# h3poteto/aws-global-accelerator-controller

Hardware: NVIDIA H100
Metric: objects reconciled/sec at 10^6 Service+Ingress; change-set bit-exact vs Go ref (higher is better)
Workload: dtype u8/u32 (bytes and indices)

## Files before the change

### aws-global-accelerator-controller_b200/csrc/gar_pipeline.h

```cpp
#pragma once

#include <stdio.h>
#include <stdlib.h>

#include <initializer_list>

#include "gar_rows.h"

#if defined(__CUDA_ARCH__)
#define GAR_ATOMIC_ADD(p, v) atomicAdd((p), (v))
#else
#define GAR_ATOMIC_ADD(p, v) (*(p) += (v))
#endif


enum Slot {
  S_DERIVED, S_OFLAGS, S_OKEY_HASH, S_STAGE_GA, S_STAGE_R53, S_ANN_R53, S_ANN_NAME, S_ANN_TAGS, S_ANN_LISTEN, S_DPORT_BEGIN, S_DPORTS,
  S_TOK_CODE, S_TOK_NAME, S_TOK_REGION,
  S_ACC_FLAGS, S_ACC_OWNER_KEY, S_ACC_OWNER, S_ACC_THOST, S_ACC_MANAGED, S_ACC_OWNER_HASH, S_ACC_THOST_HASH, S_REC_NAME_HASH, S_VAL_KEY_HASH,
  S_REC_ZONE, S_VAL_REC, S_VAL_CLS, S_VAL_KEY, S_VAL_ORPHAN, S_VAL_LINK, S_ACC_DIGEST,
  S_R53_MODE, S_R53_ACC, S_R53_ACC_DNS, S_PAIR_BEGIN, S_PAIR_OBJ, S_PAIR_HN, S_PAIR_CODE, S_PAIR_ZONE, S_PAIR_REC,
  S_IX_LB, S_IX_OWNER = S_IX_LB + 3, S_IX_THOST = S_IX_OWNER + 3, S_IX_ZONE = S_IX_THOST + 3, S_IX_VAL = S_IX_ZONE + 3,
  S_IX_ALIAS = S_IX_VAL + 3, S_IX_OBJ = S_IX_ALIAS + 3, S_IX_OVN = S_IX_OBJ + 3,
  S_SORT_KEYS = S_IX_OVN + 3, S_SORT_VALS, S_SORT_KEYS_ALT, S_SORT_VALS_ALT, S_SORT_TAGS,
  S_COUNTS, S_STATUS_GA, S_STATUS_R53, S_OPS, S_ERRFLAG, S_IX_EG, S_IX_EG_ENT, S_IX_EG_PAD, S_ACC_CLAIMED,
  S_IXA_BEGIN, S_IXA_FILL, S_IXA_ENT, S_IXA_MULTI, S_OVN_FILL, S_OVN_MULTI, S_LB_HASH, S_REC_FLAGS,
  S_NSLOTS
};


struct FClassify {
  DevTables T;
  Work W;
  u32 *derived_public;
  u8 *oflags;
  u32 *errflag;
  GAR_HD void operator()(u32 i) const {
    classify_object(T, W, i);
    u32 dv = W.derived[i];
    if (dv & OBJ_KEY_BAD) GAR_ATOMIC_ADD(errflag, 1u);
    derived_public[i] = dv & 0xFFu;
  }
};
struct FTokenise {
  DevTables T;
  Work W;
  static constexpr int kStageCols = 1;
  static constexpr u32 kStageBytes = 24 * 1024;
  static constexpr bool kStageByDefault = true;
  GAR_HD void operator()(u32 i) const { tokenise_hostname(T, W, i); }
  GAR_HD const u8 *stage_slab(int) const { return T.o.slab; }
  GAR_HD bool stage_window(int, u32 r0, u32 r1, u64 *lo, u64 *hi) const {
    gar_str a = T.o.lbi_hostname[r0], b = T.o.lbi_hostname[r1 - 1];
    *lo = GAR_STR_OFF(a);
    *hi = GAR_STR_OFF(b) + GAR_STR_LEN(b);
    return true;
  }
  template <class View>
  GAR_HD void run(u32 i, const View &view) const { tokenise_hostname_at(T, W, i, view(0, T.o.lbi_hostname[i])); }
};
struct FDigestAccel {
  DevTables T;
  Work W;
  GAR_HD void operator()(u32 i) const { digest_accelerator(T, W, i); }
};
struct FExpand {
  const u32 *begin;
  u32 nparents;
  u32 *parent_of;
  GAR_HD void operator()(u32 c) const {
    u32 lo = 0, hi = nparents;
    while (hi - lo > 1) {
      u32 mid = (lo + hi) >> 1;
      if (begin[mid] <= c) lo = mid;
      else hi = mid;
    }
    parent_of[c] = lo;
  }
};
constexpr u32 REC_INLINE_VALUES = 32;
constexpr u32 REC_HUGE_VALUES = 4096;
struct DirectView {
  const u8 *slab;
  GAR_HD Str operator()(int, gar_str r) const { return mkstr(slab, r); }
};
struct FPrepareRecord {
  DevTables T;
  Work W;
  u32 *big, *huge;
  static constexpr int kStageCols = 2;
  static constexpr u32 kStageBytes = 16 * 1024;
  static constexpr bool kStageByDefault = true;
  GAR_HD const u8 *stage_slab(int) const { return T.a.slab; }
  GAR_HD bool stage_window(int c, u32 r0, u32 r1, u64 *lo, u64 *hi) const {
    if (c == 0) {
      gar_str a = T.a.rec_name[r0], b = T.a.rec_name[r1 - 1];
      *lo = GAR_STR_OFF(a);
      *hi = GAR_STR_OFF(b) + GAR_STR_LEN(b);
      return true;
    }
    u32 v0 = T.a.rec_val_begin[r0], v1 = T.a.rec_val_begin[r1];
    if (v1 == v0) return false;
    gar_str a = T.a.val_value[v0], b = T.a.val_value[v1 - 1];
    *lo = GAR_STR_OFF(a);
    *hi = GAR_STR_OFF(b) + GAR_STR_LEN(b);
    return true;
  }
  GAR_HD void operator()(u32 r) const { run(r, DirectView{T.a.slab}); }
  template <class View>
  GAR_HD void run(u32 r, const View &view) const {
    u32 lo = 0, hi = T.a.n_zones;
    while (hi - lo > 1) {
      u32 mid = (lo + hi) >> 1;
      if (T.a.zone_rec_begin[mid] <= r) lo = mid;
      else hi = mid;
    }
    W.rec_zone[r] = lo;
    const Str nm = view(0, T.a.rec_name[r]);
    const u64 nh = gar_hash(nm);
    W.rec_name_hash[r] = nh;
    W.rec_flags[r] = find_byte(nm, 0, '\\') < nm.n ? 1 : 0;
    if (T.a.rec_has_alias[r]) ix_count(W.hist[IX_ALIAS], key_hash_zoned_h(lo, nh));
    u32 v0 = T.a.rec_val_begin[r], v1 = T.a.rec_val_begin[r + 1];
    if (v1 - v0 > REC_INLINE_VALUES) {
      u32 *list = v1 - v0 > REC_HUGE_VALUES ? huge : big;
#if defined(__CUDA_ARCH__)
      list[1 + atomicAdd(list, 1u)] = r;
#else
      list[1 + list[0]++] = r;
#endif
      return;
    }
    for (u32 v = v0; v < v1; v++) {
      W.val_rec[v] = r;
      classify_value_at(T, W, v, view(1, T.a.val_value[v]));
    }
  }
};
constexpr u32 BIG_BLOCKS = 528;
struct FClassifyBigRecords {
  DevTables T;
  Work W;
  const u32 *big, *huge;
  GAR_HD void operator()(u32 i) const {
    const u32 blk = i >> 8, tid = i & 255u, nbig = big[0], nhuge = huge[0];
    for (u32 k = blk; k < nbig; k += BIG_BLOCKS) {
      u32 r = big[1 + k];
      for (u32 v = T.a.rec_val_begin[r] + tid; v < T.a.rec_val_begin[r + 1]; v += 256) {
        W.val_rec[v] = r;
        classify_value(T, W, v);
      }
    }
    for (u32 k = 0; k < nhuge; k++) {
      u32 r = huge[1 + k];
      for (u32 v = T.a.rec_val_begin[r] + i; v < T.a.rec_val_begin[r + 1]; v += BIG_BLOCKS * 256) {
        W.val_rec[v] = r;
        classify_value(T, W, v);
      }
    }
  }
};
struct FJsonCount {
  DevTables T;
  Work W;
  GAR_HD void operator()(u32 i) const {
    u32 n = 0;
    if (W.derived[i] & GAR_DV_PORTS_FROM_ANN) {
      u32 stk[GAR_JSON_STACK_WORDS];
      int c = json_listen_ports(mkstr(T.o.slab, W.ann_listen[i]), nullptr, stk);
      n = c < 0 ? 0u : (u32)c;
    }
    W.dport_begin[i] = n;
  }
};
struct FJsonWrite {
  DevTables T;
  Work W;
  GAR_HD void operator()(u32 i) const {
    if (!(W.derived[i] & GAR_DV_PORTS_FROM_ANN)) return;
    if (W.dport_begin[i + 1] == W.dport_begin[i] || W.dport_begin[i + 1] > W.dport_cap) return;
    u32 stk[GAR_JSON_STACK_WORDS];
    json_listen_ports(mkstr(T.o.slab, W.ann_listen[i]), W.dports + W.dport_begin[i], stk);
  }
};

struct FLbHash {
  DevTables T;
  Work W;
  GAR_HD void operator()(u32 i) const {
    u64 h = key_hash_lb(mkstr(T.a.slab, T.a.lb_region[i]), mkstr(T.a.slab, T.a.lb_name[i]));
    W.lb_hash[i] = h;
    ix_count(W.hist[IX_LB], h);
  }
};
struct FRowLb {
  DevTables T;
  Work W;
  GAR_HD bool make(u32 i, u64 *h, IdxEntry *e) const {
    *h = W.lb_hash[i];
    e->a0 = T.a.lb_state[i];
    e->a1 = 0;
    e->s0 = T.a.lb_name[i];
    e->s1 = T.a.lb_region[i];
    return true;
  }
};
struct FRowOwner {
  DevTables T;
  Work W;
  GAR_HD bool make(u32 i, u64 *h, IdxEntry *e) const {
    u32 fl = W.acc_flags[i];
    *h = W.acc_owner_hash[i];
    e->a0 = fl;
    e->a1 = 0;
    e->s0 = W.acc_owner_key[i];
    e->s1 = 0;
    return (fl & ACC_MINE) && (fl & ACC_OWNER_KEYED) && i < W.acc_guest_from;
  }
};
struct FRowThost {
  DevTables T;
  Work W;
  GAR_HD bool make(u32 i, u64 *h, IdxEntry *e) const {
    *h = W.acc_thost_hash[i];
    e->a0 = e->a1 = 0;
    e->s0 = W.acc_thost[i];
    e->s1 = T.a.acc_dns[i];
    return (W.acc_flags[i] & ACC_MINE) != 0 && (!W.sharded || i >= W.acc_guest_from);
  }
};
struct FRowZone {
  DevTables T;
  GAR_HD bool make(u32 i, u64 *h, IdxEntry *e) const {
    Str zn = mkstr(T.a.slab, T.a.zone_name[i]);
    bool valid = zn.n >= 1 && zn.p[zn.n - 1] == '.';
    *h = valid ? key_hash_str(substr(zn, 0, zn.n - 1)) : 0;
    e->a0 = e->a1 = 0;
    e->s0 = T.a.zone_name[i];
    e->s1 = 0;
    return valid;
  }
};
struct FZoneLenMask {
  DevTables T;
  Work W;
  unsigned long long *mask;
  GAR_HD void operator()(u32 z) const {
    Str zn = mkstr(T.a.slab, T.a.zone_name[z]);
    if (zn.n < 1 || zn.p[zn.n - 1] != '.') return;
    ix_count(W.hist[IX_ZONE], key_hash_str(substr(zn, 0, zn.n - 1)));
    u32 b = zn.n - 1 < 255 ? zn.n - 1 : 255;
#if defined(__CUDA_ARCH__)
    atomicOr(&mask[b >> 6], 1ull << (b & 63));
#else
    mask[b >> 6] |= 1ull << (b & 63);
#endif
  }
};
struct FRowVal {
  DevTables T;
  Work W;
  GAR_HD bool make(u32 v, u64 *h, IdxEntry *e) const {
    u32 cls = W.val_cls[v];
    *h = W.val_key_hash[v];
    if (cls == VAL_NOT_OWNER) return false;
    u32 rec = W.val_rec[v];
    u32 kind = (cls & VAL_OWNER_INGRESS) ? 1u : 0u;
    u32 bs = (W.rec_flags[rec] & 1) ? VALNAME_HAS_BACKSLASH : 0u;
    e->a0 = rec;
    e->a1 = W.rec_zone[rec] | bs | (kind << 31);
    e->s0 = W.val_key[v];
    e->s1 = T.a.rec_name[rec];
    return true;
  }
};
struct FRowAlias {
  DevTables T;
  Work W;
  GAR_HD bool make(u32 r, u64 *h, IdxEntry *e) const {
    *h = key_hash_zoned_h(W.rec_zone[r], W.rec_name_hash[r]);
    e->a0 = W.rec_zone[r];
    e->a1 = T.a.rec_type[r];
    e->s0 = T.a.rec_name[r];
    e->s1 = T.a.rec_alias_dns[r];
    return T.a.rec_has_alias[r] != 0;
  }
};
struct FRowObj {
  DevTables T;
  Work W;
  GAR_HD bool make(u32 i, u64 *h, IdxEntry *e) const {
    gar_str ns = T.o.obj_ns[i];
    *h = W.okey_hash[i];
    e->a0 = T.o.obj_kind[i];
    e->a1 = 0;
    e->s0 = GAR_STR(GAR_STR_OFF(ns), GAR_STR_LEN(ns) + 1 + GAR_STR_LEN(T.o.obj_name[i]));
    e->s1 = 0;
    return !(W.derived[i] & OBJ_KEY_BAD);
  }
};
struct FRowOvn {
  DevTables T;
  Work W;
  GAR_HD bool make(u32 v, u64 *h, IdxEntry *e) const {
    u32 rec = W.val_rec[v];
    *h = key_hash_zoned_h(W.rec_zone[rec], W.rec_name_hash[rec]);
    e->a0 = rec;
    e->a1 = W.rec_zone[rec];
    e->s0 = T.a.rec_name[rec];
    e->s1 = T.a.val_value[v];
    return W.val_orphan[v] != 0;
  }
};

constexpr u32 IDX_SMALL_BUCKET = 48;
template <class RowF>
struct FIdxRows {
  RowF rowf;
  u32 *keys, *vals;
  IdxEntry *tmp;
  u32 *counts;
  u32 mask, nb;
  GAR_HD void operator()(u32 i) const {
    u64 h = 0;
    IdxEntry e;
    bool valid = rowf.make(i, &h, &e);
    u32 k = valid ? hash_bucket(h, mask) : nb;
    keys[i] = k;
    if (vals) vals[i] = i;
    if (valid) {
      e.tag = hash_tag(h);
      e.row = i;
      tmp[i] = e;
      GAR_ATOMIC_ADD(&counts[k], 1u);
    }
  }
};
struct FIdxPlace {
  const u32 *keys;
  u32 *cursor;
  const IdxEntry *tmp;
  IdxEntry *ent;
  u32 nb;
  GAR_HD void operator()(u32 i) const {
    u32 k = keys[i];
    if (k == nb) return;
#if defined(__CUDA_ARCH__)
    u32 pos = atomicAdd(&cursor[k], 1u);
#else
    u32 pos = cursor[k]++;
#endif
    ent[pos] = tmp[i];
  }
};
struct FIdxOrder {
  const u32 *begin;
  IdxEntry *ent;
  u32 *overflow;
  GAR_HD void operator()(u32 b) const {
    u32 lo = begin[b], m = begin[b + 1] - lo;
    if (m < 2) return;
    if (m > IDX_SMALL_BUCKET) {
      GAR_ATOMIC_ADD(overflow, 1u);
      return;
    }
    for (u32 k = 1; k < m; k++) {
      IdxEntry x = ent[lo + k];
      u32 j = k;
      while (j > 0 && ent[lo + j - 1].row > x.row) {
        ent[lo + j] = ent[lo + j - 1];
        j--;
      }
      if (j != k) ent[lo + j] = x;
    }
  }
};
struct FIdxGather {
  const u32 *vals;
  const u32 *nvalid;
  const IdxEntry *tmp;
  IdxEntry *ent;
  GAR_HD void operator()(u32 p) const {
    if (p < *nvalid) ent[p] = tmp[vals[p]];
  }
};
template <class RowF>
struct FIdxPlaceDirect {
  RowF rowf;
  u32 *cursor;
  IdxEntry *ent;
  u32 mask;
  GAR_HD void operator()(u32 i) const {
    u64 h = 0;
    IdxEntry e;
    if (!rowf.make(i, &h, &e)) return;
    const u32 k = hash_bucket(h, mask);
#if defined(__CUDA_ARCH__)
    const u32 pos = atomicAdd(&cursor[k], 1u);
#else
    const u32 pos = cursor[k]++;
#endif
    e.tag = hash_tag(h);
    e.row = i;
    ent[pos] = e;
  }
};
struct FIdxMultiList {
  const u32 *begin;
  u32 *multi;
  GAR_HD void operator()(u32 b) const {
    const bool m = begin[b + 1] - begin[b] >= 2;
#if defined(__CUDA_ARCH__)
    const unsigned active = __activemask();
    const unsigned votes = __ballot_sync(active, m);
    if (!m) return;
    const unsigned lane = threadIdx.x & 31u;
    const int leader = __ffs(votes) - 1;
    u32 base = 0;
    if ((int)lane == leader) base = atomicAdd(multi, (u32)__popc(votes));
    base = __shfl_sync(votes, base, leader);
    multi[1 + base + __popc(votes & ((1u << lane) - 1u))] = b;
#else
    if (m) multi[1 + multi[0]++] = b;
#endif
  }
};
struct FIdxOrderMulti {
  const u32 *begin;
  IdxEntry *ent;
  const u32 *multi;
  u32 *overflow;
  GAR_HD void operator()(u32 t) const {
    const u32 b = multi[1 + t];
    const u32 lo = begin[b], m = begin[b + 1] - lo;
    if (m > IDX_SMALL_BUCKET) {
      GAR_ATOMIC_ADD(overflow, 1u);
      return;
    }
    for (u32 k = 1; k < m; k++) {
      IdxEntry x = ent[lo + k];
      u32 j = k;
      while (j > 0 && ent[lo + j - 1].row > x.row) {
        ent[lo + j] = ent[lo + j - 1];
        j--;
      }
      if (j != k) ent[lo + j] = x;
    }
  }
};
enum FlagWord { FW_BAD_KEYS = 0, FW_IDX_OVERFLOW = 1, FW_NDPORTS = 2, FW_NPAIRS = 3, FW_SEC0 = 4 , FW_WORDS = 16 };
struct FGatherFinal {
  const u32 *src;
  u32 idx[5];
  const u32 *npairs;
  u32 *flags;
  GAR_HD void operator()(u32 k) const {
    if (k < 5) flags[FW_SEC0 + k] = src[idx[k]];
    else if (npairs) flags[FW_NPAIRS] = *npairs;
  }
};
struct FGather5 {
  const u32 *src;
  u32 idx[5];
  const u32 *extra;
  u32 *dst;
  GAR_HD void operator()(u32 k) const { dst[k] = k < 5 ? src[idx[k]] : *extra; }
};
#define GAR_RETRY_WITH_RADIX 1000
#define GAR_REFUSE_EMPTY_CACHE 1001
struct FGatherHeader {
  const u32 *ndports;
  u32 *flags;
  GAR_HD void operator()(u32) const { flags[FW_NDPORTS] = *ndports; }
};
struct FValueJoins {
  DevTables T;
  Work W;
  GAR_HD void operator()(u32 v) const {
    link_value_alias(T, W, v);
    mark_orphan_value(T, W, v);
  }
};
struct FMarkOrphanValue {
  DevTables T;
  Work W;
  GAR_HD void operator()(u32 v) const { mark_orphan_value(T, W, v); }
};

struct CountLayout {
  u32 n, nacc, nrec, nval;
  GAR_HD u32 ga_obj(u32 i) const { return i; }
  GAR_HD u32 ga_orph(u32 a) const { return n + a; }
  GAR_HD u32 r53_obj(u32 i) const { return n + nacc + i; }
  GAR_HD u32 base0() const { return 2 * n + nacc; }
  GAR_HD u32 base1() const { return 2 * n + nacc + nrec; }
  GAR_HD u32 total() const { return 2 * n + nacc + nrec + nval; }
};
constexpr u32 OPS_STAGE_CAP = 4;
struct FGaObj {
  DevTables T;
  Work W;
  u32 *counts;
  gar_op *stage;
  u32 *status;
  const u32 *rows;
  GAR_HD void operator()(u32 t, bool valid) const {
    u32 i = (rows && valid) ? rows[t] : t;
    OpSink s{stage + (size_t)t * OPS_STAGE_CAP, 0, OPS_STAGE_CAP};
    u32 st = ga_reconcile(T, W, i, valid, s);
    if (valid) {
      status[t] = st;
      counts[t] = s.n;
    }
  }
};
struct FR53Obj {
  DevTables T;
  Work W;
  u32 *counts;
  gar_op *stage;
  u32 *status;
  const u32 *rows;
  GAR_HD void operator()(u32 t, bool valid) const {
    u32 i = (rows && valid) ? rows[t] : t;
    OpSink s{stage + (size_t)t * OPS_STAGE_CAP, 0, OPS_STAGE_CAP};
    u32 prev = (valid && W.r53_mode[i] == R53_MODE_DONE) ? status[t] : 0;
    u32 st = r53_combine(T, W, i, t, valid, prev, s);
    if (valid) {
      status[t] = st;
      counts[t] = s.n;
    }
  }
};
struct FR53Prepare {
  DevTables T;
  Work W;
  u32 *status;
  const u32 *rows;
  GAR_HD void operator()(u32 t, bool valid) const { r53_prepare(T, W, (rows && valid) ? rows[t] : t, t, valid, status); }
};
struct FR53FillPairs {
  DevTables T;
  Work W;
  const u32 *rows;
  GAR_HD void operator()(u32 t) const { r53_fill_pairs(T, W, rows ? rows[t] : t, t); }
};
struct FR53Pair {
  DevTables T;
  Work W;
  GAR_HD void operator()(u32 p, bool valid) const { r53_pair(T, W, p, valid); }
};
struct DelKeys {
  const u8 *kind;
  const gar_str *key;
  const u8 *slab;
};
struct FDelKeyGa {
  DevTables T;
  Work W;
  DelKeys D;
  u32 *counts;
  gar_op *ops;
  u32 cap;
  GAR_HD void operator()(u32 k) const {
    u32 kind = D.kind[k];
    Str key = mkstr(D.slab, D.key[k]);
    if (ops && counts[k + 1] > cap) return;
    OpSink s{ops ? ops + counts[k] : nullptr, 0, 0xFFFFFFFFu};
    OwnerIter it = owner_open(W, key_hash_kinded(kind, key), key);
    for (u32 acc; (acc = owner_next(T, W, kind, it)) != GAR_NONE;) put_delete_chain(T, s, GAR_NONE, 0, acc);
    if (!ops) counts[k] = s.n;
  }
};
struct FDelKeyR53 {
  DevTables T;
  Work W;
  DelKeys D;
  u32 *counts;
  gar_op *ops;
  u32 cap;
  GAR_HD void operator()(u32 k) const {
    u32 kind = D.kind[k];
    Str key = mkstr(D.slab, D.key[k]);
    if (ops && counts[k + 1] > cap) return;
    OpSink s{ops ? ops + counts[k] : nullptr, 0, 0xFFFFFFFFu};
    Owned ow;
    owned_collect(T, W, key_hash_kinded(kind, key), kind, key, ow);
    r53_cleanup(T, W, GAR_NONE, 0, ow, s);
    if (!ops) counts[k] = s.n;
  }
};
struct FRowKnownEg {
  gar_bindings b;
  GAR_HD bool make(u32 i, u64 *h, IdxEntry *e) const {
    *h = gar_hash(mkstr(b.slab, b.known_eg_arn[i]));
    e->a0 = e->a1 = 0;
    e->s0 = b.known_eg_arn[i];
    e->s1 = 0;
    return true;
  }
};
struct FEgb {
  DevTables T;
  Work W;
  DevBindings B;
  u32 *counts;
  gar_op *ops;
  u32 *status;
  u32 cap;
  GAR_HD void operator()(u32 k) const {
    if (ops && counts[k + 1] > cap) return;
    OpSink s{ops ? ops + counts[k] : nullptr, 0, 0xFFFFFFFFu};
    u32 st = egb_reconcile(T, W, B, k, s);
    if (ops) status[k] = st;
    else counts[k] = s.n;
  }
};
struct FGatherDerived {
  const u32 *derived, *rows;
  u32 *out;
  GAR_HD void operator()(u32 t) const { out[t] = derived[rows[t]] & 0xFFu; }
};
struct FCompactOps {
  DevTables T;
  Work W;
  const u32 *scanned;
  const gar_op *stage;
  gar_op *ops;
  u32 ctrl;
  const u32 *rows;
  u32 cap;
  GAR_HD void operator()(u32 t, bool valid) const {
    u32 i = (rows && valid) ? rows[t] : t;
    u32 off = 0, c = 0;
    if (valid) {
      off = scanned[t];
      c = scanned[t + 1] - off;
      if (off > cap || c > cap - off) c = 0;
      if (c <= OPS_STAGE_CAP)
        for (u32 k = 0; k < c; k++) ops[off + k] = stage[(size_t)t * OPS_STAGE_CAP + k];
    }
    bool redo = valid && c > OPS_STAGE_CAP;
    if (GAR_ANY(redo)) {
      OpSink s{ops + off, 0, redo ? c : 0u};
      if (ctrl == GAR_CTRL_GA) ga_reconcile(T, W, i, redo, s);
      else r53_reconcile(T, W, i, redo, s);
    }
  }
};
struct FGaOrphan {
  DevTables T;
  Work W;
  CountLayout L;
  u32 *counts;
  gar_op *ops;
  u32 cap;
  GAR_HD void operator()(u32 a) const {
    if (ops && counts[L.ga_orph(a) + 1] == counts[L.ga_orph(a)]) return;
    if (ops && counts[L.ga_orph(a) + 1] > cap) return;
    OpSink s{ops ? ops + counts[L.ga_orph(a)] : nullptr, 0, 0xFFFFFFFFu};
    ga_orphan(T, W, a, s);
    if (!ops) counts[L.ga_orph(a)] = s.n;
  }
};
struct FR53OrphanAlias {
  DevTables T;
  Work W;
  CountLayout L;
  u32 *counts;
  gar_op *ops;
  u32 cap;
  GAR_HD void operator()(u32 r) const {
    if (!ops) {
      OpSink s{nullptr, 0, 0};
      r53_orphan_alias(T, W, r, s);
      counts[L.base0() + r] = s.n;
      return;
    }
    if (counts[L.base0() + r + 1] == counts[L.base0() + r]) return;
    if (counts[L.total()] > cap) return;
    u32 z = W.rec_zone[r];
    u32 zv = T.a.rec_val_begin[T.a.zone_rec_begin[z]];
    u32 off = counts[L.base0()] + (counts[L.base1() + zv] - counts[L.base1()]) + (counts[L.base0() + r] - counts[L.base0()]);
    OpSink s{ops + off, 0, 0xFFFFFFFFu};
    r53_orphan_alias(T, W, r, s);
  }
};
struct FR53OrphanValue {
  DevTables T;
  Work W;
  CountLayout L;
  u32 *counts;
  gar_op *ops;
  u32 cap;
  GAR_HD void operator()(u32 v) const {
    if (!ops) {
      counts[L.base1() + v] = W.val_orphan[v];
      return;
    }
    if (!W.val_orphan[v] || counts[L.total()] > cap) return;
    u32 r = W.val_rec[v];
    u32 z = W.rec_zone[r];
    u32 rend = T.a.zone_rec_begin[z + 1];
    u32 off = counts[L.base0()] + (counts[L.base0() + rend] - counts[L.base0()]) + (counts[L.base1() + v] - counts[L.base1()]);
    gar_op o;
    o.head = GAR_OP_HEAD(GAR_OP_R53_DELETE_RECORD, GAR_CTRL_R53, 0);
    o.obj = GAR_NONE;
    o.sub = 1;
    o.a0 = z;
    o.a1 = r;
    o.a2 = v;
    ops[off] = o;
  }
};


struct DiffCounts {
  u64 n_ops;
  u64 section_begin[GAR_N_SECTIONS + 1];
  u64 n_dports;
  u32 bad_keys;
};

GAR_HD u32 next_pow2(u32 x) {
  u32 p = 1;
  while (p < x) p <<= 1;
  return p;
}
inline int ilog2(u32 p) {
  int b = 0;
  while ((1u << b) < p) b++;
  return b;
}

template <class B>
struct Pipeline {
  B &be;
  DevTables T;
  Work W{};
  bool force_radix = false;
  explicit Pipeline(B &b, const DevTables &t) : be(b), T(t) {}

  template <class RowF>
  HashIdx build_index(int slot, u32 nrows, u32 load, RowF rowf, u32 *overflow, bool force_radix) {
    u32 nb = next_pow2(nrows / load < 16 ? 16 : nrows / load);
    u32 *keys = (u32 *)be.ensure(S_SORT_KEYS, sizeof(u32) * (size_t)(nrows + 1));
    u32 *vals = (u32 *)be.ensure(S_SORT_VALS, sizeof(u32) * (size_t)(nrows + 1));
    IdxEntry *tmp = (IdxEntry *)be.ensure(S_SORT_TAGS, sizeof(IdxEntry) * (size_t)(nrows + 1));
    u32 *begin = (u32 *)be.ensure(slot + 0, sizeof(u32) * (size_t)(nb + 2));
    IdxEntry *ent = (IdxEntry *)be.ensure(slot + 1, sizeof(IdxEntry) * (size_t)(nrows + 1));
    be.fill32(begin, 0, nb + 2);
    if (nrows) be.for_each("idx_rows", nrows, FIdxRows<RowF>{rowf, keys, force_radix ? vals : nullptr, tmp, begin, nb - 1, nb});
    be.exclusive_scan(begin, nb + 2);
    if (nrows && !force_radix) {
      u32 *cursor = (u32 *)be.ensure(S_SORT_KEYS_ALT, sizeof(u32) * (size_t)(nb + 1));
      be.copy32(cursor, begin, nb);
      be.for_each("idx_place", nrows, FIdxPlace{keys, cursor, tmp, ent, nb});
      be.for_each("idx_order", nb, FIdxOrder{begin, ent, overflow});
    } else if (nrows) {
      u32 *keys2 = (u32 *)be.ensure(S_SORT_KEYS_ALT, sizeof(u32) * (size_t)(nrows + 1));
      u32 *vals2 = (u32 *)be.ensure(S_SORT_VALS_ALT, sizeof(u32) * (size_t)(nrows + 1));
      be.sort_pairs(keys, vals, keys2, vals2, nrows, ilog2(nb) + 1);
      be.for_each("idx_gather", nrows, FIdxGather{vals, begin + nb, tmp, ent});
    }
    return HashIdx{begin, ent, nb - 1};
  }

  bool prepared = false;
  u64 n_dports = 0;
  u32 *errflag = nullptr;

  u32 acc_guest_from = 0xFFFFFFFFu;
  u32 sharded = 0;
  bool orphan_sweep = true;
  bool allow_empty_cache = false;

  void alloc_obj_work() {
    const u32 n = T.o.n_objects, nlbi = T.o.n_lbi;
    W.derived = (u32 *)be.ensure(S_DERIVED, 4 * (size_t)(n + 1));
    W.okey_hash = (u64 *)be.ensure(S_OKEY_HASH, 8 * (size_t)(n + 1));
    W.ann_r53 = (gar_str *)be.ensure(S_ANN_R53, 8 * (size_t)(n + 1));
    W.ann_name = (gar_str *)be.ensure(S_ANN_NAME, 8 * (size_t)(n + 1));
    W.ann_tags = (gar_str *)be.ensure(S_ANN_TAGS, 8 * (size_t)(n + 1));
    W.ann_listen = (gar_str *)be.ensure(S_ANN_LISTEN, 8 * (size_t)(n + 1));
    W.dport_begin = (u32 *)be.out_dport_begin(n);
    W.tok_code = (u8 *)be.out_tok_code(nlbi);
    W.tok_name = (gar_str *)be.out_tok_name(nlbi);
    W.tok_region = (gar_str *)be.out_tok_region(nlbi);
    W.r53_mode = (u8 *)be.ensure(S_R53_MODE, (size_t)n + 1);
    W.r53_acc = (u32 *)be.ensure(S_R53_ACC, 4 * (size_t)(n + 1));
    W.r53_acc_dns = (gar_str *)be.ensure(S_R53_ACC_DNS, 8 * (size_t)(n + 1));
  }
  void alloc_work() {
    const u32 nacc = T.a.n_accels, nrec = T.a.n_records, nval = T.a.n_values;
    alloc_obj_work();
    W.acc_flags = (u32 *)be.ensure(S_ACC_FLAGS, 4 * (size_t)(nacc + 1));
    W.acc_owner_key = (gar_str *)be.ensure(S_ACC_OWNER_KEY, 8 * (size_t)(nacc + 1));
    W.acc_owner = (gar_str *)be.ensure(S_ACC_OWNER, 8 * (size_t)(nacc + 1));
    W.acc_thost = (gar_str *)be.ensure(S_ACC_THOST, 8 * (size_t)(nacc + 1));
    W.acc_managed = (gar_str *)be.ensure(S_ACC_MANAGED, 8 * (size_t)(nacc + 1));
    W.acc_owner_hash = (u64 *)be.ensure(S_ACC_OWNER_HASH, 8 * (size_t)(nacc + 1));
    W.acc_thost_hash = (u64 *)be.ensure(S_ACC_THOST_HASH, 8 * (size_t)(nacc + 1));
    W.rec_name_hash = (u64 *)be.ensure(S_REC_NAME_HASH, 8 * (size_t)(nrec + 1));
    W.val_key_hash = (u64 *)be.ensure(S_VAL_KEY_HASH, 8 * (size_t)(nval + 1));
    W.rec_zone = (u32 *)be.ensure(S_REC_ZONE, 4 * (size_t)(nrec + 1));
    W.val_rec = (u32 *)be.ensure(S_VAL_REC, 4 * (size_t)(nval + 1));
    W.val_cls = (u8 *)be.ensure(S_VAL_CLS, nval + 1);
    W.val_key = (gar_str *)be.ensure(S_VAL_KEY, 8 * (size_t)(nval + 1));
    W.val_orphan = (u8 *)be.ensure(S_VAL_ORPHAN, nval + 1);
    W.val_link = (ValLink *)be.ensure(S_VAL_LINK, sizeof(ValLink) * (size_t)(nval + 1));
    W.acc_digest = (AccDigest *)be.ensure(S_ACC_DIGEST, sizeof(AccDigest) * (size_t)(nacc + 1));
    W.lb_hash = (u64 *)be.ensure(S_LB_HASH, 8 * (size_t)(T.a.n_lbs + 1));
    W.rec_flags = (u8 *)be.ensure(S_REC_FLAGS, (size_t)nrec + 1);
    for (int k = 0; k < IX_N; k++) W.hist[k] = IxHist{nullptr, 0};
    W.pair_cap = 0;
    W.dport_cap = 0;
    errflag = (u32 *)be.ensure(S_ERRFLAG, 256);
    be.fill32(errflag, 0, FW_WORDS);
    W.acc_guest_from = acc_guest_from;
    W.sharded = sharded;
    W.acc_claimed = nullptr;
  }
  void stage1() {
    const u32 n = T.o.n_objects, nlbi = T.o.n_lbi, nacc = T.a.n_accels, nrec = T.a.n_records, nval = T.a.n_values;
    u32 *derived_public = (u32 *)be.out_derived(n);
    if (n) be.for_each("classify_objects", n, FClassify{T, W, derived_public, nullptr, errflag});
    if (nlbi) be.for_each_staged("tokenise_hostnames", nlbi, FTokenise{T, W});
    if (nacc) be.for_each("digest_accelerators", nacc, FDigestAccel{T, W});
    if (T.a.n_lbs) be.for_each("hash_load_balancers", T.a.n_lbs, FLbHash{T, W});
    {
      unsigned long long *zm = (unsigned long long *)(errflag + 16 + 8);
      be.fill32((u32 *)zm, 0, 8);
      if (T.a.n_zones) be.for_each("zone_len_mask", T.a.n_zones, FZoneLenMask{T, W, zm});
      W.zone_len_mask = (const u64 *)zm;
    }
    if (nrec) {
      u32 *big = (u32 *)be.ensure(S_SORT_KEYS, 4 * (size_t)(nval / REC_INLINE_VALUES + 2));
      u32 *huge = (u32 *)be.ensure(S_SORT_VALS, 4 * (size_t)(nval / REC_HUGE_VALUES + 2));
      be.fill32(big, 0, 1);
      be.fill32(huge, 0, 1);
      be.for_each_staged("prepare_records", nrec, FPrepareRecord{T, W, big, huge});
      if (nval > REC_INLINE_VALUES) be.for_each("prepare_records", BIG_BLOCKS * 256, FClassifyBigRecords{T, W, big, huge});
    }
  }
  struct IxPlan {
    u32 off[IX_N] = {}, nb[IX_N] = {}, rows[IX_N] = {};
    bool want[IX_N] = {};
    u32 total_nb = 0;
    u64 total_rows = 0;
  };
  IxPlan planA;
  u32 *ixa_begin = nullptr, *ixa_fill = nullptr, *ixa_multi = nullptr;
  IdxEntry *ixa_ent = nullptr;
  u32 ovn_nb = 0;
  void arm_group_a(u32 want_mask) {
    const u32 rows[IX_N] = {T.a.n_lbs, T.a.n_accels, T.a.n_accels, T.a.n_zones, T.a.n_values, T.a.n_records, T.o.n_objects, 0};
    const u32 load[IX_N] = {1, 1, 1, 1, 1, 2, 1, 8};
    planA = IxPlan{};
    for (int k = 0; k < IX_OVN; k++) {
      planA.want[k] = (want_mask >> k) & 1u;
      if (!planA.want[k]) continue;
      planA.rows[k] = rows[k];
      planA.nb[k] = next_pow2(rows[k] / load[k] < 16 ? 16 : rows[k] / load[k]);
      planA.off[k] = planA.total_nb;
      planA.total_nb += planA.nb[k];
      planA.total_rows += rows[k];
    }
    ixa_begin = (u32 *)be.ensure(S_IXA_BEGIN, 4 * (size_t)(planA.total_nb + 2));
    be.fill32(ixa_begin, 0, (size_t)planA.total_nb + 2);
    for (int k = 0; k < IX_OVN; k++)
      if (planA.want[k]) W.hist[k] = IxHist{ixa_begin + planA.off[k], planA.nb[k] - 1};
  }
  HashIdx group_a_index(int k) const { return HashIdx{ixa_begin + planA.off[k], ixa_ent, planA.nb[k] - 1}; }
  template <class RowF>
  FIdxPlaceDirect<RowF> placer(int k, RowF rowf) const {
    return FIdxPlaceDirect<RowF>{rowf, ixa_fill + planA.off[k], ixa_ent, planA.nb[k] - 1};
  }
  void finish_group_a() {
    u32 *overflow = errflag + FW_IDX_OVERFLOW;
    be.exclusive_scan(ixa_begin, planA.total_nb + 1);
    ixa_fill = (u32 *)be.ensure(S_IXA_FILL, 4 * (size_t)(planA.total_nb + 1));
    ixa_ent = (IdxEntry *)be.ensure(S_IXA_ENT, sizeof(IdxEntry) * (size_t)(planA.total_rows + 1));
    const u32 multi_cap = (u32)(planA.total_rows / 2 + 1);
    ixa_multi = (u32 *)be.ensure(S_IXA_MULTI, 4 * (size_t)(multi_cap + 2));
    be.copy32(ixa_fill, ixa_begin, (size_t)planA.total_nb + 1);
    be.fill32(ixa_multi, 0, 1);
    const IxPlan &P = planA;
    auto n = [&](int k) { return P.want[k] ? P.rows[k] : 0u; };
    be.for_each_multi("idx_place", {n(IX_LB), n(IX_OWNER), n(IX_THOST), n(IX_ZONE), n(IX_VAL), n(IX_ALIAS), n(IX_OBJ), P.total_nb},
                      placer(IX_LB, FRowLb{T, W}), placer(IX_OWNER, FRowOwner{T, W}), placer(IX_THOST, FRowThost{T, W}), placer(IX_ZONE, FRowZone{T}),
                      placer(IX_VAL, FRowVal{T, W}), placer(IX_ALIAS, FRowAlias{T, W}), placer(IX_OBJ, FRowObj{T, W}), FIdxMultiList{ixa_begin, ixa_multi});
    be.for_each_dyn("idx_order", ixa_multi, multi_cap, FIdxOrderMulti{ixa_begin, ixa_ent, ixa_multi, overflow});
    if (P.want[IX_LB]) W.ix_lb = group_a_index(IX_LB);
    if (P.want[IX_OWNER]) W.ix_owner = group_a_index(IX_OWNER);
    if (P.want[IX_THOST]) W.ix_thost = group_a_index(IX_THOST);
    if (P.want[IX_ZONE]) W.ix_zone = group_a_index(IX_ZONE);
    if (P.want[IX_VAL]) W.ix_val = group_a_index(IX_VAL);
    if (P.want[IX_ALIAS]) W.ix_alias = group_a_index(IX_ALIAS);
    if (P.want[IX_OBJ]) W.ix_obj = group_a_index(IX_OBJ);
  }
  void arm_ovn() {
    ovn_nb = next_pow2(T.a.n_values / 8 < 16 ? 16 : T.a.n_values / 8);
    u32 *cnt = (u32 *)be.ensure(S_IX_OVN + 0, 4 * (size_t)(ovn_nb + 2));
    be.fill32(cnt, 0, (size_t)ovn_nb + 2);
    W.hist[IX_OVN] = IxHist{cnt, ovn_nb - 1};
  }
  void finish_ovn() {
    const u32 nval = T.a.n_values;
    u32 *begin = W.hist[IX_OVN].cnt;
    be.exclusive_scan(begin, ovn_nb + 1);
    u32 *cursor = (u32 *)be.ensure(S_OVN_FILL, 4 * (size_t)(ovn_nb + 1));
    IdxEntry *ent = (IdxEntry *)be.ensure(S_IX_OVN + 1, sizeof(IdxEntry) * (size_t)(nval + 1));
    u32 *multi = (u32 *)be.ensure(S_OVN_MULTI, 4 * (size_t)(nval / 2 + 3));
    be.copy32(cursor, begin, (size_t)ovn_nb + 1);
    be.fill32(multi, 0, 1);
    be.for_each_multi("idx_place", {nval, ovn_nb}, FIdxPlaceDirect<FRowOvn>{FRowOvn{T, W}, cursor, ent, ovn_nb - 1}, FIdxMultiList{begin, multi});
    be.for_each_dyn("idx_order", multi, nval / 2 + 1, FIdxOrderMulti{begin, ent, multi, errflag + FW_IDX_OVERFLOW});
    W.ix_ovn = HashIdx{begin, ent, ovn_nb - 1};
  }

  void prepare_route() {
    alloc_work();
    arm_group_a(1u << IX_ALIAS);
    stage1();
    finish_group_a();
  }
  void prepare_directory() {
    alloc_work();
    arm_group_a((1u << IX_LB) | (1u << IX_THOST));
    if (T.o.n_lbi) be.for_each("tokenise_hostnames", T.o.n_lbi, FTokenise{T, W});
    if (T.a.n_accels) be.for_each("digest_accelerators", T.a.n_accels, FDigestAccel{T, W});
    if (T.a.n_lbs) be.for_each("hash_load_balancers", T.a.n_lbs, FLbHash{T, W});
    finish_group_a();
  }

  u32 dport_cap = 0, pair_cap = 0;
  u64 ops_cap = 0;
  bool tiny_caps = false;
  int prepare() {
    const u32 n = T.o.n_objects, nacc = T.a.n_accels, nzone = T.a.n_zones, nrec = T.a.n_records, nval = T.a.n_values;
    alloc_work();
    if (!force_radix) {
      arm_group_a((1u << IX_OVN) - 1);
      arm_ovn();
    }
    stage1();
    listen_ports();

    u32 *overflow = errflag + FW_IDX_OVERFLOW;
    if (!force_radix) {
      finish_group_a();
      if (nval) be.for_each("value_joins", nval, FValueJoins{T, W});
      finish_ovn();
    } else {
      W.ix_lb = build_index(S_IX_LB, T.a.n_lbs, 1, FRowLb{T, W}, overflow, true);
      W.ix_owner = build_index(S_IX_OWNER, nacc, 1, FRowOwner{T, W}, overflow, true);
      W.ix_thost = build_index(S_IX_THOST, nacc, 1, FRowThost{T, W}, overflow, true);
      W.ix_zone = build_index(S_IX_ZONE, nzone, 1, FRowZone{T}, overflow, true);
      W.ix_val = build_index(S_IX_VAL, nval, 1, FRowVal{T, W}, overflow, true);
      W.ix_alias = build_index(S_IX_ALIAS, nrec, 2, FRowAlias{T, W}, overflow, true);
      W.ix_obj = build_index(S_IX_OBJ, n, 1, FRowObj{T, W}, overflow, true);
      if (nval) be.for_each("value_joins", nval, FValueJoins{T, W});
      W.ix_ovn = build_index(S_IX_OVN, nval, 8, FRowOvn{T, W}, overflow, true);
    }
    obj_stale = ovn_stale = false;
    return GAR_OK;
  }
  void listen_ports() {
    const u32 n = T.o.n_objects;
    be.fill32(W.dport_begin, 0, (size_t)n + 1);
    if (n) be.for_each("listen_ports_count", n, FJsonCount{T, W});
    be.exclusive_scan(W.dport_begin, n + 1);
    be.for_each("gather_header", 1, FGatherHeader{W.dport_begin + n, errflag});
    if (dport_cap < n / 2 + 1024 && !(tiny_caps && dport_cap)) dport_cap = tiny_caps ? 1 : n / 2 + 1024;
    W.dport_cap = dport_cap;
    W.dports = (i32 *)be.out_dports(dport_cap);
    if (n) be.for_each("listen_ports_write", n, FJsonWrite{T, W});
  }

  bool obj_stale = false, ovn_stale = false;
  void prepare_objects() {
    const u32 n = T.o.n_objects, nlbi = T.o.n_lbi;
    alloc_obj_work();
    be.fill32(errflag, 0, FW_WORDS);
    W.hist[IX_OBJ] = IxHist{nullptr, 0};
    u32 *derived_public = (u32 *)be.out_derived(n);
    if (n) be.for_each("classify_objects", n, FClassify{T, W, derived_public, nullptr, errflag});
    if (nlbi) be.for_each_staged("tokenise_hostnames", nlbi, FTokenise{T, W});
    listen_ports();
    W.ix_obj = build_index(S_IX_OBJ, n, 1, FRowObj{T, W}, errflag + FW_IDX_OVERFLOW, force_radix);
    obj_stale = false;
    ovn_stale = true;
  }
  void prepare_orphan_values() {
    const u32 nval = T.a.n_values;
    if (!force_radix) {
      arm_ovn();
      if (nval) be.for_each("orphan_values", nval, FMarkOrphanValue{T, W});
      finish_ovn();
    } else {
      W.hist[IX_OVN] = IxHist{nullptr, 0};
      if (nval) be.for_each("orphan_values", nval, FMarkOrphanValue{T, W});
      W.ix_ovn = build_index(S_IX_OVN, nval, 8, FRowOvn{T, W}, errflag + FW_IDX_OVERFLOW, true);
    }
    ovn_stale = false;
  }
  int index_objects() {
    for (int attempt = 0; attempt < 2; attempt++) {
      if (!prepared) prepare();
      else if (obj_stale) prepare_objects();
      prepared = true;
      u32 fl[FW_WORDS];
      be.download(fl, errflag, sizeof(fl));
      if (fl[FW_BAD_KEYS]) return GAR_E_INVALID;
      if (fl[FW_IDX_OVERFLOW] && !force_radix) {
        force_radix = true;
        prepared = false;
        continue;
      }
      return GAR_OK;
    }
    return GAR_E_STATE;
  }

  u64 n_pairs = 0;
  void r53_relational(u32 slots, const u32 *rows, u32 *st_r53) {
    W.pair_begin = (u32 *)be.ensure(S_PAIR_BEGIN, 4 * (size_t)(slots + 2));
    be.fill32(W.pair_begin, 0, (size_t)slots + 1);
    if (slots) be.for_each_warp("r53_prepare", slots, FR53Prepare{T, W, st_r53, rows});
    be.exclusive_scan(W.pair_begin, slots + 1);
    if (pair_cap < slots + slots / 2 + 1024 && !(tiny_caps && pair_cap)) pair_cap = tiny_caps ? 1 : slots + slots / 2 + 1024;
    W.pair_cap = pair_cap;
    W.pair_obj = (u32 *)be.ensure(S_PAIR_OBJ, 4 * (size_t)(pair_cap + 1));
    W.pair_hn = (gar_str *)be.ensure(S_PAIR_HN, 8 * (size_t)(pair_cap + 1));
    W.pair_code = (u8 *)be.ensure(S_PAIR_CODE, (size_t)pair_cap + 1);
    W.pair_zone = (u32 *)be.ensure(S_PAIR_ZONE, 4 * (size_t)(pair_cap + 1));
    W.pair_rec = (u32 *)be.ensure(S_PAIR_REC, 4 * (size_t)(pair_cap + 1));
    if (slots) {
      be.for_each("r53_fill_pairs", slots, FR53FillPairs{T, W, rows});
      be.for_each_warp_dyn("r53_pairs", W.pair_begin + slots, pair_cap, FR53Pair{T, W});
    }
  }

  template <class OpsAlloc>
  int decide_all(OpsAlloc ops_alloc) {
    const u32 n = T.o.n_objects, nacc = T.a.n_accels, nrec = T.a.n_records, nval = T.a.n_values;
    CountLayout L{n, nacc, nrec, nval};
    u32 *counts = (u32 *)be.ensure(S_COUNTS, 4 * (size_t)(L.total() + 2));
    be.fill32(counts, 0, (size_t)L.total() + 1);
    gar_op *stage_ga = (gar_op *)be.ensure(S_STAGE_GA, sizeof(gar_op) * ((size_t)n * OPS_STAGE_CAP + 1));
    gar_op *stage_r53 = (gar_op *)be.ensure(S_STAGE_R53, sizeof(gar_op) * ((size_t)n * OPS_STAGE_CAP + 1));
    u32 *st_ga = (u32 *)be.out_status_ga(n);
    u32 *st_r53 = (u32 *)be.out_status_r53(n);
    W.acc_claimed = (u8 *)be.ensure(S_ACC_CLAIMED, (size_t)nacc + 4);
    be.fill32((u32 *)W.acc_claimed, 0, ((size_t)nacc + 3) / 4);
    if (n) be.for_each_warp("ga_objects", n, FGaObj{T, W, counts + L.ga_obj(0), stage_ga, st_ga, nullptr});
    r53_relational(n, nullptr, st_r53);
    if (n) be.for_each_warp("r53_objects", n, FR53Obj{T, W, counts + L.r53_obj(0), stage_r53, st_r53, nullptr});
    if (orphan_sweep)
      be.for_each_multi("orphans_count", {nacc, nrec, nval}, FGaOrphan{T, W, L, counts, nullptr, 0}, FR53OrphanAlias{T, W, L, counts, nullptr, 0},
                        FR53OrphanValue{T, W, L, counts, nullptr, 0});
    be.exclusive_scan(counts, L.total() + 1);
    be.for_each("gather_section_begins", 6, FGatherFinal{counts, {0, L.ga_orph(0), L.r53_obj(0), L.base0(), L.total()}, W.pair_begin + n, errflag});

    const u64 est = tiny_caps ? 1 : (u64)n + nacc / 8 + 1024;
    if (ops_cap < est) ops_cap = est;
    gar_op *ops = (gar_op *)ops_alloc(ops_cap);
    const u32 cap = ops_cap > 0xFFFFFFF0ull ? 0xFFFFFFF0u : (u32)ops_cap;
    if (n) be.for_each_warp("ga_objects_compact", n, FCompactOps{T, W, counts + L.ga_obj(0), stage_ga, ops, GAR_CTRL_GA, nullptr, cap});
    if (n) be.for_each_warp("r53_objects_compact", n, FCompactOps{T, W, counts + L.r53_obj(0), stage_r53, ops, GAR_CTRL_R53, nullptr, cap});
    if (orphan_sweep)
      be.for_each_multi("orphans_emit", {nacc, nrec, nval}, FGaOrphan{T, W, L, counts, ops, cap}, FR53OrphanAlias{T, W, L, counts, ops, cap},
                        FR53OrphanValue{T, W, L, counts, ops, cap});
    W.acc_claimed = nullptr;
    return GAR_OK;
  }

  template <class OpsAlloc>
  int decide_keys(const u32 *rows, u32 m, DelKeys D, u32 nd, OpsAlloc ops_alloc) {
    const u32 total = 2 * m + 2 * nd;
    u32 *counts = (u32 *)be.ensure(S_COUNTS, 4 * (size_t)(total + 2));
    be.fill32(counts, 0, (size_t)total + 1);
    u32 *c_ga = counts, *c_gad = counts + m, *c_r53 = counts + m + nd, *c_r53d = counts + 2 * m + nd;
    gar_op *stage_ga = (gar_op *)be.ensure(S_STAGE_GA, sizeof(gar_op) * ((size_t)m * OPS_STAGE_CAP + 1));
    gar_op *stage_r53 = (gar_op *)be.ensure(S_STAGE_R53, sizeof(gar_op) * ((size_t)m * OPS_STAGE_CAP + 1));
    u32 *st_ga = (u32 *)be.out_status_ga(m);
    u32 *st_r53 = (u32 *)be.out_status_r53(m);
    u32 *derived_out = (u32 *)be.out_derived_keys(m);
    if (m) {
      be.for_each("gather_derived", m, FGatherDerived{W.derived, rows, derived_out});
      be.for_each_warp("ga_objects", m, FGaObj{T, W, c_ga, stage_ga, st_ga, rows});
    }
    if (nd) be.for_each("ga_deleted_keys_count", nd, FDelKeyGa{T, W, D, c_gad, nullptr, 0});
    r53_relational(m, rows, st_r53);
    if (m) be.for_each_warp("r53_objects", m, FR53Obj{T, W, c_r53, stage_r53, st_r53, rows});
    if (nd) be.for_each("r53_deleted_keys_count", nd, FDelKeyR53{T, W, D, c_r53d, nullptr, 0});
    be.exclusive_scan(counts, total + 1);
    be.for_each("gather_section_begins", 6, FGatherFinal{counts, {0, m, m + nd, 2 * m + nd, total}, W.pair_begin + m, errflag});
    const u64 est = tiny_caps ? 1 : 2 * (u64)m + 4 * (u64)nd + 256;
    if (ops_cap < est) ops_cap = est;
    gar_op *ops = (gar_op *)ops_alloc(ops_cap);
    const u32 cap = ops_cap > 0xFFFFFFF0ull ? 0xFFFFFFF0u : (u32)ops_cap;
    if (m) be.for_each_warp("ga_objects_compact", m, FCompactOps{T, W, c_ga, stage_ga, ops, GAR_CTRL_GA, rows, cap});
    if (nd) be.for_each("ga_deleted_keys_emit", nd, FDelKeyGa{T, W, D, c_gad, ops, cap});
    if (m) be.for_each_warp("r53_objects_compact", m, FCompactOps{T, W, c_r53, stage_r53, ops, GAR_CTRL_R53, rows, cap});
    if (nd) be.for_each("r53_deleted_keys_emit", nd, FDelKeyR53{T, W, D, c_r53d, ops, cap});
    return GAR_OK;
  }

  template <class OpsAlloc>
  int decide_bindings(const gar_bindings &b, OpsAlloc ops_alloc) {
    u32 *overflow = errflag + FW_IDX_OVERFLOW;
    const u32 nb = b.n_bindings;
    DevBindings DB{b, build_index(S_IX_EG, b.n_known_egs, 1, FRowKnownEg{b}, overflow, force_radix)};
    u32 *counts = (u32 *)be.ensure(S_COUNTS, 4 * (size_t)(nb + 2));
    be.fill32(counts, 0, (size_t)nb + 1);
    u32 *st = (u32 *)be.out_status_ga(nb);
    if (nb) be.for_each("egb_count", nb, FEgb{T, W, DB, counts, nullptr, nullptr, 0});
    be.exclusive_scan(counts, nb + 1);
    be.for_each("gather_section_begins", 6, FGatherFinal{counts, {0, nb, nb, nb, nb}, nullptr, errflag});
    const u64 est = tiny_caps ? 1 : 4 * (u64)nb + 256;
    if (ops_cap < est) ops_cap = est;
    gar_op *ops = (gar_op *)ops_alloc(ops_cap);
    const u32 cap = ops_cap > 0xFFFFFFF0ull ? 0xFFFFFFF0u : (u32)ops_cap;
    if (nb) be.for_each("egb_emit", nb, FEgb{T, W, DB, counts, ops, st, cap});
    return GAR_OK;
  }

  template <class DecideF>
  int run_with(DiffCounts *dc, bool full, DecideF decide) {
    for (int attempt = 0; attempt < 8; attempt++) {
      u64 sig = 0;
      if (full) {
        sig = hmix(hmix(prepared ? (obj_stale || ovn_stale ? 9 : 1) : 2, force_radix ? 3 : 4), hmix(hmix(dport_cap, pair_cap), ops_cap));
        sig = hmix(sig, hmix(orphan_sweep ? 5 : 6, tiny_caps ? 7 : 8)) | 1;
      }
      const int g = full ? be.graph_begin(sig) : 0;
      int rc = GAR_OK;
      if (g != 2) {
        if (!prepared) rc = prepare();
        else if (obj_stale) prepare_objects();
        if (rc == GAR_OK && full && ovn_stale) prepare_orphan_values();
        if (rc == GAR_OK) rc = decide();
      }
      prepared = true;
      if (full) be.graph_end();
      if (rc != GAR_OK) return rc;
      u32 fl[FW_WORDS];
      be.download(fl, errflag, sizeof(fl));
      if (fl[FW_BAD_KEYS]) return GAR_E_INVALID;
      if (fl[FW_IDX_OVERFLOW] && !force_radix) {
        force_radix = true;
        prepared = false;
        continue;
      }
      if (fl[FW_NDPORTS] > dport_cap) {
        dport_cap = fl[FW_NDPORTS] + fl[FW_NDPORTS] / 8 + 16;
        prepared = false;
        continue;
      }
      if (fl[FW_NPAIRS] > pair_cap) {
        pair_cap = fl[FW_NPAIRS] + fl[FW_NPAIRS] / 8 + 16;
        continue;
      }
      const u64 nops = fl[FW_SEC0 + 4];
      if (nops > ops_cap) {
        ops_cap = nops + nops / 8 + 16;
        continue;
      }
      n_dports = fl[FW_NDPORTS];
      n_pairs = fl[FW_NPAIRS];
      for (int k = 0; k < 5; k++) dc->section_begin[k] = fl[FW_SEC0 + k];
      dc->n_ops = nops;
      dc->n_dports = full ? n_dports : 0;
      if (full && T.o.n_objects == 0 && !sharded && !allow_empty_cache && nops != 0) return GAR_REFUSE_EMPTY_CACHE;
      return GAR_OK;
    }
    return GAR_E_STATE;
  }
  template <class OpsAlloc>
  int run(DiffCounts *dc, OpsAlloc ops_alloc) {
    return run_with(dc, true, [&] { return decide_all(ops_alloc); });
  }
  template <class OpsAlloc>
  int run_keys(const u32 *rows, u32 m, DelKeys D, u32 nd, DiffCounts *dc, OpsAlloc ops_alloc) {
    return run_with(dc, false, [&] { return decide_keys(rows, m, D, nd, ops_alloc); });
  }
  template <class OpsAlloc>
  int run_bindings(const gar_bindings &b, DiffCounts *dc, OpsAlloc ops_alloc) {
    return run_with(dc, false, [&] { return decide_bindings(b, ops_alloc); });
  }
};
```

### aws-global-accelerator-controller_b200/csrc/gar_rows.h

```cpp
#pragma once

#include "gar_common.h"
#include "gar_json.h"


struct DevTables {
  gar_objects o;
  gar_actual a;
  const u8 *cluster;
  u32 cluster_len;
};

enum {
  OBJ_HAS_NAME_ANN = 1u << 8,
  OBJ_HAS_TAGS_ANN = 1u << 9,
  OBJ_KEY_BAD = 1u << 10,
};

enum {
  ACC_MINE = 1u << 0,
  ACC_OWNER_KEYED = 1u << 1,
  ACC_OWNER_INGRESS = 1u << 2,
  ACC_OWNER_3PART = 1u << 3,
  ACC_HAS_MANAGED = 1u << 4, ACC_HAS_OWNER = 1u << 5, ACC_HAS_THOST = 1u << 6,
};

enum {
  R53_MODE_DONE = 0,
  R53_MODE_PAIRS = 1,
  R53_MODE_OBJECT = 2,
};
enum { PAIR_IN_SYNC = 0, PAIR_CREATE = 1, PAIR_UPSERT = 2, PAIR_NO_ZONE = 3,
       PAIR_REPEAT = 4 };
#define VALNAME_HAS_BACKSLASH (1u << 30)

enum { VAL_NOT_OWNER = 0, VAL_OWNER_SERVICE = 1, VAL_OWNER_INGRESS = 2, VAL_OWNER_3PART = 4 };

struct alignas(64) AccDigest {
  u32 flags;
  u32 lis;
  u32 eg;
  u32 pr_begin;
  u32 ep_begin;
  u16 n_ports, n_eps;
  i32 port0, port1;
  gar_str name;
  gar_str thost;
  gar_str owner_key;
  gar_str ep0;
};
enum {
  ACCD_ENABLED = 1u << 8,
  ACCD_MANAGED_TRUE = 1u << 9,
  ACCD_LIS_NONE = 1u << 10, ACCD_LIS_MANY = 1u << 11,
  ACCD_LIS_UDP = 1u << 12,
  ACCD_EG_NONE = 1u << 13, ACCD_EG_MANY = 1u << 14,
};
struct alignas(16) ValLink {
  u32 alias_row, pad;
  gar_str alias_dns;
};

enum IxId { IX_LB, IX_OWNER, IX_THOST, IX_ZONE, IX_VAL, IX_ALIAS, IX_OBJ, IX_OVN, IX_N };
struct IxHist {
  u32 *cnt;
  u32 mask;
};
#if defined(__CUDA_ARCH__)
#define GAR_HIST_ADD(p) atomicAdd((p), 1u)
#else
#define GAR_HIST_ADD(p) (++*(p))
#endif
GAR_HD void ix_count(const IxHist &h, u64 key_hash) {
  if (h.cnt) GAR_HIST_ADD(&h.cnt[(u32)key_hash & h.mask]);
}

struct Work {
  IxHist hist[IX_N];
  u64 *lb_hash;
  u8 *rec_flags;
  u32 pair_cap;
  u32 dport_cap;
  u32 *derived;
  u64 *okey_hash;
  gar_str *ann_r53;
  gar_str *ann_name;
  gar_str *ann_tags;
  gar_str *ann_listen;
  u32 *dport_begin;
  i32 *dports;
  u8 *tok_code;
  gar_str *tok_name, *tok_region;
  u32 *acc_flags;
  gar_str *acc_owner_key;
  gar_str *acc_owner;
  gar_str *acc_thost;
  gar_str *acc_managed;
  AccDigest *acc_digest;
  u64 *acc_owner_hash;
  u64 *acc_thost_hash;
  u32 *rec_zone;
  u64 *rec_name_hash;
  u32 *val_rec;
  u8 *val_cls;
  gar_str *val_key;
  u64 *val_key_hash;
  u8 *val_orphan;
  ValLink *val_link;
  u32 acc_guest_from;
  u32 sharded;
  u8 *acc_claimed;
  u8 *r53_mode;
  u32 *r53_acc;
  gar_str *r53_acc_dns;
  u32 *pair_begin;
  u32 *pair_obj;
  gar_str *pair_hn;
  u8 *pair_code;
  u32 *pair_zone;
  u32 *pair_rec;
  HashIdx ix_lb;
  HashIdx ix_owner;
  HashIdx ix_thost;
  HashIdx ix_zone;
  const u64 *zone_len_mask;
  HashIdx ix_val;
  HashIdx ix_alias;
  HashIdx ix_obj;
  HashIdx ix_ovn;
};

GAR_HD bool acc_in_owner_index(const Work &W, u32 a, u32 fl) { return (fl & ACC_MINE) && (fl & ACC_OWNER_KEYED) && a < W.acc_guest_from; }
GAR_HD bool acc_in_thost_index(const Work &W, u32 a, u32 fl) { return (fl & ACC_MINE) != 0 && (!W.sharded || a >= W.acc_guest_from); }


GAR_HD u64 key_hash_kinded(u32 kind, Str nsname) { return hmix(kind + 1, gar_hash(nsname)); }
GAR_HD u64 key_hash_lb(Str region, Str name) { return hmix(gar_hash(region), gar_hash(name)); }
GAR_HD u64 key_hash_zoned_h(u32 zone, u64 name_hash) { return hmix((u64)zone + 0x100, name_hash); }
GAR_HD u64 key_hash_zoned(u32 zone, Str name) { return key_hash_zoned_h(zone, gar_hash(name)); }
GAR_HD u64 key_hash_str(Str s) { return gar_hash(s); }

GAR_HD Str object_key(const DevTables &T, u32 i) {
  gar_str ns = T.o.obj_ns[i], nm = T.o.obj_name[i];
  return Str{T.o.slab + GAR_STR_OFF(ns), GAR_STR_LEN(ns) + 1 + GAR_STR_LEN(nm)};
}
GAR_HD bool object_key_ok(const DevTables &T, u32 i) {
  gar_str ns = T.o.obj_ns[i], nm = T.o.obj_name[i];
  u64 sep = GAR_STR_OFF(ns) + GAR_STR_LEN(ns);
  return GAR_STR_OFF(nm) == sep + 1 && sep < T.o.slab_len && T.o.slab[sep] == '/';
}


#define ANN_PREFIX "aws-global-accelerator-controller.h3poteto.dev/"

GAR_HD bool proto_is(Str p, char a, char b, char c) {
  return p.n == 3 && (p.p[0] | 0x20) == a && (p.p[1] | 0x20) == b && (p.p[2] | 0x20) == c;
}

GAR_HD void classify_object(const DevTables &T, const Work &W, u32 i) {
  const gar_objects &o = T.o;
  u32 kind = o.obj_kind[i];
  u32 dv = 0;
  bool has_lbtype = false, has_ingclass = false;
  gar_str r53 = 0, name = 0, tags = 0, listen = 0;
  bool has_listen = false;
  for (u32 k = o.obj_ann_begin[i]; k < o.obj_ann_begin[i + 1]; k++) {
    Str key = mkstr(o.slab, o.ann_key[k]);
    gar_str vref = o.ann_val[k];
    if (HAS_PREFIX_LIT(key, ANN_PREFIX)) {
      Str t = substr(key, sizeof(ANN_PREFIX) - 1, key.n - (u32)(sizeof(ANN_PREFIX) - 1));
      if (STREQ_LIT(t, "global-accelerator-managed")) {
        dv |= GAR_DV_GA_MANAGED;
      } else if (STREQ_LIT(t, "route53-hostname")) {
        dv |= GAR_DV_R53_ANNOTATED;
        r53 = vref;
      } else if (STREQ_LIT(t, "client-ip-preservation")) {
        if (STREQ_LIT(mkstr(o.slab, vref), "true")) dv |= GAR_DV_IP_PRESERVE;
        else dv &= ~(u32)GAR_DV_IP_PRESERVE;
      } else if (STREQ_LIT(t, "global-accelerator-name")) {
        dv |= OBJ_HAS_NAME_ANN;
        name = vref;
      } else if (STREQ_LIT(t, "global-accelerator-tags")) {
        dv |= OBJ_HAS_TAGS_ANN;
        tags = vref;
      } else if (STREQ_LIT(t, "ip-address-type")) {
        Str v = mkstr(o.slab, vref);
        if (STREQ_LIT(v, "ipv4") || STREQ_LIT(v, "IPV4")) dv |= GAR_DV_IPV4;
        else dv &= ~(u32)GAR_DV_IPV4;
      }
    } else if (STREQ_LIT(key, "service.beta.kubernetes.io/aws-load-balancer-type")) {
      has_lbtype = true;
    } else if (STREQ_LIT(key, "kubernetes.io/ingress.class")) {
      has_ingclass = true;
    } else if (STREQ_LIT(key, "alb.ingress.kubernetes.io/listen-ports")) {
      has_listen = true;
      listen = vref;
    }
  }
  if (kind == GAR_KIND_SERVICE) {
    bool lbsvc = o.obj_spec_type[i] == GAR_SVC_LOADBALANCER && (has_lbtype || (o.obj_flags[i] & GAR_OBJ_HAS_LB_CLASS));
    if (lbsvc) dv |= GAR_DV_GA_ELIGIBLE | GAR_DV_R53_ELIGIBLE;
    bool udp = false;
    for (u32 p = o.obj_port_begin[i]; p < o.obj_port_begin[i + 1]; p++) {
      Str pr = mkstr(o.slab, o.port_proto[p]);
      if (proto_is(pr, 'u', 'd', 'p')) udp = true;
      else if (proto_is(pr, 't', 'c', 'p')) udp = false;
    }
    if (udp) dv |= GAR_DV_PROTO_UDP;
  } else {
    bool alb = has_ingclass;
    if ((o.obj_flags[i] & GAR_OBJ_HAS_INGRESS_CLASS) && STREQ_LIT(mkstr(o.slab, o.obj_ingress_class[i]), "alb")) alb = true;
    if (alb) dv |= GAR_DV_GA_ELIGIBLE;
    dv |= GAR_DV_R53_ELIGIBLE;
    if (has_listen) dv |= GAR_DV_PORTS_FROM_ANN;
  }
  if (!object_key_ok(T, i)) dv |= OBJ_KEY_BAD;
  const u64 okh = (dv & OBJ_KEY_BAD) ? 0 : key_hash_kinded(kind, object_key(T, i));
  W.okey_hash[i] = okh;
  if (!(dv & OBJ_KEY_BAD)) ix_count(W.hist[IX_OBJ], okh);
  W.derived[i] = dv;
  W.ann_r53[i] = r53;
  W.ann_name[i] = name;
  W.ann_tags[i] = tags;
  W.ann_listen[i] = listen;
}


GAR_HD u32 name_dash_id(Str s) {
  u32 last = GAR_NONE;
  for (u32 i = 0; i < s.n; i += 8) {
    u64 w = load_word(s, i);
    u64 pad = s.n - i < 8 ? ~lowmask(s.n - i) & 0x8080808080808080ull : 0;
    if (w & 0x8080808080808080ull) return 0;
    u64 dash = swar_eq_exact(w, '-') & ~pad;
    u64 ok = swar_in_range(w, '0', '9') | swar_in_range(w, 'A', 'Z') | swar_in_range(w, 'a', 'z') | swar_eq_exact(w, '_') | dash | pad;
    if (ok != 0x8080808080808080ull) return 0;
    if (dash) last = i + ((63 - clz64(dash)) >> 3);
  }
  if (last == GAR_NONE || last < 1 || last + 1 >= s.n) return 0;
  return last;
}

GAR_HD u8 tokenise_str(Str h, u64 base, gar_str *name_out, gar_str *region_out) {
  u8 code;
  gar_str name = 0, region = 0;
  u32 d1 = find_byte(h, 0, '.');
  u32 d2 = d1 < h.n ? find_byte(h, d1 + 1, '.') : h.n;
  u32 d3 = d2 < h.n ? find_byte(h, d2 + 1, '.') : h.n;
  if (d1 >= h.n) {
    code = GAR_TOK_PANIC;
  } else if (!(STREQ_LIT(h, "amazonaws.com") || HAS_SUFFIX_LIT(h, ".amazonaws.com"))) {
    code = GAR_TOK_NOT_AWS;
  } else if (HAS_SUFFIX_LIT(h, ".elb.amazonaws.com")) {
    Str sub = substr(h, 0, d1);
    region = GAR_STR(base + d1 + 1, d2 - d1 - 1);
    if (HAS_PREFIX_LIT(sub, "internal-")) {
      u32 g = name_dash_id(substr(sub, 9, sub.n - 9));
      if (g) {
        code = GAR_TOK_ALB_INTERNAL;
        name = GAR_STR(base + 9, g);
      } else {
        code = GAR_TOK_ERR_INTERNAL_ALB;
      }
    } else {
      u32 g = name_dash_id(sub);
      if (g) {
        code = GAR_TOK_ALB_PUBLIC;
        name = GAR_STR(base, g);
      } else {
        code = GAR_TOK_ERR_PUBLIC_ALB;
      }
    }
  } else {
    bool nlb = false;
    if (h.n >= 20) {
      u32 last = GAR_NONE;
      for (u32 i = d1; i <= h.n - 20; i = find_byte(h, i + 1, '.'))
        if (lit_eq_at(h, i, ".elb.")) last = i;
      if (last != GAR_NONE) nlb = find_byte(substr(h, 0, h.n - 14), last + 5, '\n') >= h.n - 14;
    }
    if (!nlb) {
      code = GAR_TOK_ERR_NOT_ELB;
    } else {
      u32 g = name_dash_id(substr(h, 0, d1));
      if (g) {
        code = GAR_TOK_NLB;
        name = GAR_STR(base, g);
        region = GAR_STR(base + d2 + 1, d3 - d2 - 1);
      } else {
        code = GAR_TOK_ERR_NLB;
      }
    }
  }
  if (code > GAR_TOK_NLB) {
    name = 0;
    region = 0;
  }
  *name_out = name;
  *region_out = region;
  return code;
}
GAR_HD void tokenise_hostname_at(const DevTables &T, const Work &W, u32 row, Str h) {
  gar_str name, region;
  u8 code = tokenise_str(h, GAR_STR_OFF(T.o.lbi_hostname[row]), &name, &region);
  W.tok_code[row] = code;
  W.tok_name[row] = name;
  W.tok_region[row] = region;
}
GAR_HD void tokenise_hostname(const DevTables &T, const Work &W, u32 row) { tokenise_hostname_at(T, W, row, mkstr(T.o.slab, T.o.lbi_hostname[row])); }


#define TAG_MANAGED "aws-global-accelerator-controller-managed"
#define TAG_OWNER "aws-global-accelerator-owner"
#define TAG_THOST "aws-global-accelerator-target-hostname"
#define TAG_CLUSTER "aws-global-accelerator-cluster"

GAR_HD u32 count_slashes(Str s) { return count_byte(s, '/'); }

GAR_HD void digest_accelerator(const DevTables &T, const Work &W, u32 a) {
  const gar_actual &A = T.a;
  gar_str managed = 0, owner = 0, thost = 0, cluster = 0;
  u32 fl = 0;
  for (u32 t = A.acc_tag_begin[a]; t < A.acc_tag_begin[a + 1]; t++) {
    Str k = mkstr(A.slab, A.tag_key[t]);
    if (STREQ_LIT(k, TAG_MANAGED)) {
      managed = A.tag_val[t];
      fl |= ACC_HAS_MANAGED;
    } else if (STREQ_LIT(k, TAG_OWNER)) {
      owner = A.tag_val[t];
      fl |= ACC_HAS_OWNER;
    } else if (STREQ_LIT(k, TAG_THOST)) {
      thost = A.tag_val[t];
      fl |= ACC_HAS_THOST;
    } else if (STREQ_LIT(k, TAG_CLUSTER)) {
      cluster = A.tag_val[t];
    }
  }
  Str cl = mkstr(A.slab, cluster);
  if (STREQ_LIT(mkstr(A.slab, managed), "true") && streq(cl, Str{T.cluster, T.cluster_len})) fl |= ACC_MINE;
  Str ow = mkstr(A.slab, owner);
  gar_str key = 0;
  if (HAS_PREFIX_LIT(ow, "service/")) {
    fl |= ACC_OWNER_KEYED;
    key = GAR_STR(GAR_STR_OFF(owner) + 8, ow.n - 8);
  } else if (HAS_PREFIX_LIT(ow, "ingress/")) {
    fl |= ACC_OWNER_KEYED | ACC_OWNER_INGRESS;
    key = GAR_STR(GAR_STR_OFF(owner) + 8, ow.n - 8);
  }
  if ((fl & ACC_OWNER_KEYED) && count_slashes(mkstr(A.slab, key)) == 1) fl |= ACC_OWNER_3PART;
  AccDigest d;
  d.flags = fl | (A.acc_enabled[a] ? ACCD_ENABLED : 0) | (STREQ_LIT(mkstr(A.slab, managed), "true") ? ACCD_MANAGED_TRUE : 0);
  d.lis = d.eg = d.pr_begin = d.ep_begin = 0;
  d.n_ports = d.n_eps = 0;
  d.port0 = d.port1 = 0;
  d.ep0 = 0;
  u32 lb = A.acc_lis_begin[a], le = A.acc_lis_begin[a + 1];
  if (le == lb) d.flags |= ACCD_LIS_NONE;
  else if (le - lb > 1) d.flags |= ACCD_LIS_MANY;
  else {
    d.lis = lb;
    if (A.lis_proto[lb] == GAR_PROTO_UDP) d.flags |= ACCD_LIS_UDP;
    d.pr_begin = A.lis_pr_begin[lb];
    u32 np = A.lis_pr_begin[lb + 1] - d.pr_begin;
    d.n_ports = (u16)(np > 0xFFFF ? 0xFFFF : np);
    if (np > 0) d.port0 = A.pr_from[d.pr_begin];
    if (np > 1) d.port1 = A.pr_from[d.pr_begin + 1];
    u32 eb = A.lis_eg_begin[lb], ee = A.lis_eg_begin[lb + 1];
    if (ee == eb) d.flags |= ACCD_EG_NONE;
    else if (ee - eb > 1) d.flags |= ACCD_EG_MANY;
    else {
      d.eg = eb;
      d.ep_begin = A.eg_ep_begin[eb];
      u32 ne = A.eg_ep_begin[eb + 1] - d.ep_begin;
      d.n_eps = (u16)(ne > 0xFFFF ? 0xFFFF : ne);
      if (ne > 0) d.ep0 = A.ep_id[d.ep_begin];
    }
  }
  d.name = A.acc_name[a];
  d.thost = thost;
  d.owner_key = key;
  W.acc_digest[a] = d;
  const u64 owner_hash = (fl & ACC_OWNER_KEYED) ? key_hash_kinded((fl & ACC_OWNER_INGRESS) ? 1u : 0u, mkstr(A.slab, key)) : 0;
  const u64 thost_hash = (fl & ACC_MINE) ? gar_hash(mkstr(A.slab, thost)) : 0;
  W.acc_owner_hash[a] = owner_hash;
  W.acc_thost_hash[a] = thost_hash;
  if (acc_in_owner_index(W, a, fl)) ix_count(W.hist[IX_OWNER], owner_hash);
  if (acc_in_thost_index(W, a, fl)) ix_count(W.hist[IX_THOST], thost_hash);
  W.acc_flags[a] = fl;
  W.acc_owner_key[a] = key;
  W.acc_owner[a] = owner;
  W.acc_thost[a] = thost;
  W.acc_managed[a] = managed;
}


#define R53_HERITAGE "\"heritage=aws-global-accelerator-controller,cluster="

GAR_HD void classify_value_at(const DevTables &T, const Work &W, u32 v, Str s) {
  const gar_actual &A = T.a;
  gar_str ref = A.val_value[v];
  u8 cls = VAL_NOT_OWNER;
  gar_str key = 0;
  const u32 hl = (u32)(sizeof(R53_HERITAGE) - 1);
  u32 fixed = hl + T.cluster_len + 1 + 8 + 1;
  if (s.n >= fixed && HAS_PREFIX_LIT(s, R53_HERITAGE) && streq(substr(s, hl, T.cluster_len), Str{T.cluster, T.cluster_len}) &&
      s.p[hl + T.cluster_len] == ',' && s.p[s.n - 1] == '"') {
    u32 ro = hl + T.cluster_len + 1;
    Str rest = substr(s, ro, s.n - 1 - ro);
    if (HAS_PREFIX_LIT(rest, "service/")) cls = VAL_OWNER_SERVICE;
    else if (HAS_PREFIX_LIT(rest, "ingress/")) cls = VAL_OWNER_INGRESS;
    if (cls) {
      key = GAR_STR(GAR_STR_OFF(ref) + ro + 8, rest.n - 8);
      if (count_slashes(substr(rest, 8, rest.n - 8)) == 1) cls |= VAL_OWNER_3PART;
    }
  }
  W.val_cls[v] = cls;
  W.val_key[v] = key;
  const u64 vkh = cls ? key_hash_kinded((cls & VAL_OWNER_INGRESS) ? 1u : 0u, substr(s, (u32)(GAR_STR_OFF(key) - GAR_STR_OFF(ref)), (u32)GAR_STR_LEN(key))) : 0;
  W.val_key_hash[v] = vkh;
  if (cls) ix_count(W.hist[IX_VAL], vkh);
}
GAR_HD void classify_value(const DevTables &T, const Work &W, u32 v) { classify_value_at(T, W, v, mkstr(T.a.slab, T.a.val_value[v])); }


GAR_HD u32 find_lb(const DevTables &T, const Work &W, Str region, Str name, u32 *state) {
  Cursor c = idx_open(W.ix_lb, key_hash_lb(region, name));
  IdxEntry e;
  while (idx_next(W.ix_lb, c, &e))
    if (streq(mkstr(T.a.slab, e.s0), name) && streq(mkstr(T.a.slab, e.s1), region)) {
      *state = e.a0;
      return e.row;
    }
  return GAR_NONE;
}

struct OwnerIter {
  Cursor c;
  Str key;
};
GAR_HD OwnerIter owner_open(const Work &W, u64 key_hash, Str key) { return OwnerIter{idx_open(W.ix_owner, key_hash), key}; }
GAR_HD u32 owner_next(const DevTables &T, const Work &W, u32 kind, OwnerIter &it) {
  IdxEntry e;
  while (idx_next(W.ix_owner, it.c, &e)) {
    if ((((e.a0 & ACC_OWNER_INGRESS) != 0) ? 1u : 0u) != kind) continue;
    if (streq(mkstr(T.a.slab, e.s0), it.key)) return e.row;
  }
  return GAR_NONE;
}

GAR_HD u32 find_by_hostname(const DevTables &T, const Work &W, Str hostname, u32 *first, gar_str *first_dns) {
  Cursor c = idx_open(W.ix_thost, key_hash_str(hostname));
  u32 n = 0;
  *first = GAR_NONE;
  IdxEntry e;
  while (idx_next(W.ix_thost, c, &e)) {
    if (!streq(mkstr(T.a.slab, e.s0), hostname)) continue;
    if (n == 0) {
      *first = e.row;
      *first_dns = e.s1;
    }
    if (++n >= 2) break;
  }
  return n;
}

GAR_HD bool zone_len_possible(const Work &W, u32 n) {
  u32 b = n < 255 ? n : 255;
  return (W.zone_len_mask[b >> 6] >> (b & 63)) & 1ull;
}
GAR_HD u32 find_hosted_zone(const DevTables &T, const Work &W, Str hostname) {
  Str t = hostname;
  for (;;) {
    if (t.n == 0) return GAR_NONE;
    if (zone_len_possible(W, t.n)) {
      Cursor c = idx_open(W.ix_zone, key_hash_str(t));
      IdxEntry e;
      while (idx_next(W.ix_zone, c, &e)) {
        Str zn = mkstr(T.a.slab, e.s0);
        if (zn.n == t.n + 1 && streq(substr(zn, 0, t.n), t)) return e.row;
      }
    }
    u32 k = find_byte(t, 0, '.');
    if (k >= t.n) return GAR_NONE;
    t = substr(t, k + 1, t.n - k - 1);
  }
}

GAR_HD bool record_name_matches(Str name, Str hostname) {
  u32 w = GAR_NONE;
  for (u32 k = find_byte(name, 0, '\\'); k + 4 <= name.n; k = find_byte(name, k + 1, '\\'))
    if (name.p[k + 1] == '0' && name.p[k + 2] == '5' && name.p[k + 3] == '2') {
      w = k;
      break;
    }
  if (w == GAR_NONE) return name.n == hostname.n + 1 && name.p[name.n - 1] == '.' && streq(substr(name, 0, hostname.n), hostname);
  if (name.n - 3 != hostname.n + 1) return false;
  if (name.p[name.n - 1] != '.') return false;
  if (w >= hostname.n || hostname.p[w] != '*') return false;
  if (!streq(substr(name, 0, w), substr(hostname, 0, w))) return false;
  u32 tail = hostname.n - w - 1;
  return streq(substr(name, w + 4, tail), substr(hostname, w + 1, tail));
}


GAR_HD Cursor cursor_none() { return Cursor{0, 0, 0}; }
GAR_HD Cursor u_open(const HashIdx &ix, bool active, u64 h) { return active ? idx_open(ix, h) : cursor_none(); }

GAR_HD bool u_bucket_step(const HashIdx &ix, bool searching, Cursor &c, IdxEntry *e) {
  bool step = searching && c.pos < c.end;
  if (step) {
    *e = load_entry(ix.ent + c.pos++);
    return e->tag == c.tag;
  }
  return false;
}
#define U_BUCKET_LOOP(searching_expr, cur) for (; GAR_ANY((searching_expr) && (cur).pos < (cur).end);)

GAR_HD u32 u_find_lb(const DevTables &T, const Work &W, bool active, Str region, Str name, u32 *state) {
  u64 h = hmix(u_hash(active, region), u_hash(active, name));
  Cursor c = u_open(W.ix_lb, active, h);
  u32 found = GAR_NONE;
  U_BUCKET_LOOP(found == GAR_NONE, c) {
    IdxEntry e;
    bool hit = u_bucket_step(W.ix_lb, found == GAR_NONE, c, &e);
    bool eq = u_streq(hit, mkstr(T.a.slab, e.s0), name);
    eq = u_streq(eq, mkstr(T.a.slab, e.s1), region);
    if (eq) {
      found = e.row;
      *state = e.a0;
    }
  }
  return found;
}

GAR_HD u32 u_owner_next(const DevTables &T, const Work &W, bool active, u32 kind, Str key, Cursor &c) {
  u32 found = GAR_NONE;
  U_BUCKET_LOOP(active && found == GAR_NONE, c) {
    IdxEntry e;
    bool hit = u_bucket_step(W.ix_owner, active && found == GAR_NONE, c, &e);
    hit = hit && (((e.a0 & ACC_OWNER_INGRESS) != 0) ? 1u : 0u) == kind;
    if (u_streq(hit, mkstr(T.a.slab, e.s0), key)) found = e.row;
  }
  if (found != GAR_NONE && W.acc_claimed) W.acc_claimed[found] = 1;
  return found;
}

GAR_HD u32 u_find_by_hostname(const DevTables &T, const Work &W, bool active, Str hostname, u32 *first, gar_str *first_dns) {
  Cursor c = u_open(W.ix_thost, active, u_hash(active, hostname));
  u32 n = 0;
  *first = GAR_NONE;
  U_BUCKET_LOOP(n < 2, c) {
    IdxEntry e;
    bool hit = u_bucket_step(W.ix_thost, n < 2, c, &e);
    if (u_streq(hit, mkstr(T.a.slab, e.s0), hostname)) {
      if (n == 0) {
        *first = e.row;
        *first_dns = e.s1;
      }
      n++;
    }
  }
  return n;
}

GAR_HD u32 u_find_hosted_zone(const DevTables &T, const Work &W, bool active, Str hostname) {
  Str t = hostname;
  u32 zone = GAR_NONE;
  bool walking = active;
  for (;;) {
    bool round = walking && t.n != 0;
    if (!GAR_ANY(round)) break;
    bool probe = round && zone_len_possible(W, t.n);
    Cursor c = u_open(W.ix_zone, probe, u_hash(probe, t));
    U_BUCKET_LOOP(zone == GAR_NONE, c) {
      IdxEntry e;
      bool hit = u_bucket_step(W.ix_zone, zone == GAR_NONE, c, &e);
      Str zn = mkstr(T.a.slab, e.s0);
      hit = hit && zn.n == t.n + 1;
      if (u_streq(hit, substr(zn, 0, hit ? t.n : 0), t)) zone = e.row;
    }
    u32 k = u_find_byte(round && zone == GAR_NONE, t, 0, '.');
    if (round) {
      if (zone != GAR_NONE || k >= t.n) walking = false;
      else t = substr(t, k + 1, t.n - k - 1);
    }
  }
  return zone;
}

GAR_HD u32 u_first_alias_a(const DevTables &T, const Work &W, bool active, u32 zone, Str name, gar_str *alias_dns) {
  Cursor c = u_open(W.ix_alias, active, hmix((u64)zone + 0x100, u_hash(active, name)));
  u32 found = GAR_NONE;
  U_BUCKET_LOOP(found == GAR_NONE, c) {
    IdxEntry e;
    bool hit = u_bucket_step(W.ix_alias, found == GAR_NONE, c, &e);
    hit = hit && e.a0 == zone && e.a1 == GAR_RR_A;
    if (u_streq(hit, mkstr(T.a.slab, e.s0), name)) {
      found = e.row;
      *alias_dns = e.s1;
    }
  }
  return found;
}

GAR_HD bool u_record_name_matches(bool active, Str name, Str hostname) {
  u32 bs = u_find_byte(active, name, 0, '\\');
  bool plain = active && bs >= name.n;
  bool shape = plain && name.n == hostname.n + 1 && name.p[name.n - 1] == '.';
  bool eq = u_streq(shape, substr(name, 0, shape ? hostname.n : 0), hostname);
  if (active && !plain) eq = record_name_matches(name, hostname);
  return eq;
}


struct OpSink {
  gar_op *out;
  u32 n;
  u32 cap;
  GAR_HD void put(u32 head, u32 obj, u32 sub, u32 a0, u32 a1, u32 a2) {
    if (out && n < cap) {
      gar_op o;
      o.head = head;
      o.obj = obj;
      o.sub = sub;
      o.a0 = a0;
      o.a1 = a1;
      o.a2 = a2;
      out[n] = o;
    }
    n++;
  }
};


struct PortList {
  const i32 *p;
  u32 n;
};
GAR_HD PortList desired_ports(const DevTables &T, const Work &W, u32 i) {
  if (W.derived[i] & GAR_DV_PORTS_FROM_ANN) {
    u32 b = W.dport_begin[i], e = W.dport_begin[i + 1];
    if (e > W.dport_cap) b = e = 0;
    return PortList{W.dports + b, e - b};
  }
  u32 b = T.o.obj_port_begin[i];
  return PortList{T.o.port_number + b, T.o.obj_port_begin[i + 1] - b};
}

GAR_HD bool ports_changed(PortList l, PortList d) {
  u32 nmin = l.n < d.n ? l.n : d.n;
  u32 pre = 0;
  while (pre < nmin && l.p[pre] == d.p[pre]) pre++;
  u32 suf = 0;
  while (suf < nmin - pre && l.p[l.n - 1 - suf] == d.p[d.n - 1 - suf]) suf++;
  u32 ml = l.n - pre - suf, md = d.n - pre - suf;
  for (u32 x = 0; x < ml + md; x++) {
    i32 px = x < ml ? l.p[pre + x] : d.p[pre + (x - ml)];
    u32 cnt = 0;
    for (u32 y = 0; y < l.n && cnt < 2; y++) cnt += (l.p[y] == px);
    for (u32 y = 0; y < d.n && cnt < 2; y++) cnt += (d.p[y] == px);
    if (cnt <= 1) return true;
  }
  return false;
}

GAR_HD bool accel_name_matches(const DevTables &T, const Work &W, u32 i, u32 kind, Str acc_name) {
  if (W.derived[i] & OBJ_HAS_NAME_ANN) {
    Str n = mkstr(T.o.slab, W.ann_name[i]);
    if (n.n != 0) return streq(n, acc_name);
  }
  Str ns = mkstr(T.o.slab, T.o.obj_ns[i]), nm = mkstr(T.o.slab, T.o.obj_name[i]);
  if (acc_name.n != 7 + 1 + ns.n + 1 + nm.n) return false;
  const u64 res = kind == GAR_KIND_SERVICE ? 0x2d65636976726573ull  : 0x2d73736572676e69ull ;
  if (ld64u(acc_name.p) != res) return false;
  if (acc_name.p[8 + ns.n] != '-') return false;
  return streq(substr(acc_name, 8, ns.n), ns) && streq(substr(acc_name, 9 + ns.n, nm.n), nm);
}

GAR_HD Str actual_tag(const DevTables &T, u32 acc, Str key) {
  Str v{T.a.slab, 0};
  for (u32 t = T.a.acc_tag_begin[acc]; t < T.a.acc_tag_begin[acc + 1]; t++)
    if (streq(mkstr(T.a.slab, T.a.tag_key[t]), key)) v = mkstr(T.a.slab, T.a.tag_val[t]);
  return v;
}

struct TagPiece {
  Str key, val;
  bool ok;
};
GAR_HD TagPiece tag_piece(Str piece) {
  u32 eq = find_byte(piece, 0, '=');
  TagPiece t;
  t.ok = eq < piece.n && find_byte(piece, eq + 1, '=') >= piece.n;
  if (t.ok) {
    t.key = substr(piece, 0, eq);
    t.val = substr(piece, eq + 1, piece.n - eq - 1);
  } else {
    t.key = t.val = Str{piece.p, 0};
  }
  return t;
}
GAR_HD bool next_piece(Str all, u32 *pos, Str *piece) {
  if (*pos > all.n) return false;
  u32 b = *pos;
  u32 k = find_byte(all, b, ',');
  *piece = substr(all, b, k - b);
  *pos = k + 1;
  return true;
}

GAR_HD bool accelerator_tags_changed(const DevTables &T, const Work &W, u32 i, u32 kind, u32 acc, Str lb_dns) {
  const gar_actual &A = T.a;
  bool user_managed = false, user_owner = false, user_thost = false;
  if (W.derived[i] & OBJ_HAS_TAGS_ANN) {
    Str tags = mkstr(T.o.slab, W.ann_tags[i]);
    u32 pos = 0;
    Str piece;
    while (next_piece(tags, &pos, &piece)) {
      TagPiece tp = tag_piece(piece);
      if (!tp.ok) continue;
      if (STREQ_LIT(tp.key, TAG_MANAGED)) user_managed = true;
      else if (STREQ_LIT(tp.key, TAG_OWNER)) user_owner = true;
      else if (STREQ_LIT(tp.key, TAG_THOST)) user_thost = true;
      bool overridden = false;
      u32 pos2 = pos;
      Str piece2;
      while (next_piece(tags, &pos2, &piece2)) {
        TagPiece t2 = tag_piece(piece2);
        if (t2.ok && streq(t2.key, tp.key)) {
          overridden = true;
          break;
        }
      }
      if (overridden) continue;
      if (!streq(actual_tag(T, acc, tp.key), tp.val)) return true;
    }
  }
  u32 fl = W.acc_flags[acc];
  if (!user_managed && !STREQ_LIT(mkstr(A.slab, W.acc_managed[acc]), "true")) return true;
  if (!user_owner) {
    bool ok = (fl & ACC_OWNER_KEYED) && (((fl & ACC_OWNER_INGRESS) ? 1u : 0u) == kind) && streq(mkstr(A.slab, W.acc_owner_key[acc]), object_key(T, i));
    if (!ok) return true;
  }
  if (!user_thost && !streq(mkstr(A.slab, W.acc_thost[acc]), lb_dns)) return true;
  return false;
}

GAR_HD void put_delete_chain(const DevTables &T, OpSink &s, u32 obj, u32 kind, u32 acc) {
  const gar_actual &A = T.a;
  u32 lb = A.acc_lis_begin[acc], le = A.acc_lis_begin[acc + 1];
  u32 lis = GAR_NONE, eg = GAR_NONE;
  if (le - lb == 1) {
    lis = lb;
    u32 eb = A.lis_eg_begin[lis], ee = A.lis_eg_begin[lis + 1];
    if (ee - eb == 1) eg = eb;
  }
  s.put(GAR_OP_HEAD(GAR_OP_GA_DELETE_CHAIN, GAR_CTRL_GA, obj == GAR_NONE ? 0 : kind), obj, 0, acc, lis, eg);
}


GAR_HD bool u_accelerator_changed(const DevTables &T, const Work &W, bool act, u32 i, u32 dv, u32 kind, u32 acc, const AccDigest &d, Str okey, Str lb_dns) {
  const gar_actual &A = T.a;
  bool ch = act && !(d.flags & ACCD_ENABLED);
  bool need = act && !ch;
  Str an = need ? mkstr(A.slab, d.name) : Str{A.slab, 0};
  Str ann = (need && (dv & OBJ_HAS_NAME_ANN)) ? mkstr(T.o.slab, W.ann_name[i]) : Str{T.o.slab, 0};
  bool by_ann = need && ann.n != 0;
  bool eq_ann = u_streq(by_ann, ann, an);
  Str ns = need ? mkstr(T.o.slab, T.o.obj_ns[i]) : Str{T.o.slab, 0};
  Str nm = need ? mkstr(T.o.slab, T.o.obj_name[i]) : Str{T.o.slab, 0};
  bool shape = need && !by_ann && an.n == 9 + ns.n + nm.n &&
               ld64u(an.p) == (kind == GAR_KIND_SERVICE ? 0x2d65636976726573ull  : 0x2d73736572676e69ull ) &&
               an.p[8 + ns.n] == '-';
  bool eq_def = u_streq(shape, substr(an, 8, shape ? ns.n : 0), ns);
  eq_def = u_streq(eq_def, substr(an, 9 + ns.n, eq_def ? nm.n : 0), nm);
  if (need && !(by_ann ? eq_ann : eq_def)) ch = true;
  bool tagcheck = act && !ch;
  bool overlay = tagcheck && (dv & OBJ_HAS_TAGS_ANN);
  if (overlay) ch = accelerator_tags_changed(T, W, i, kind, acc, lb_dns);
  bool sys = tagcheck && !overlay;
  u32 fl = d.flags;
  if (sys && !(fl & ACCD_MANAGED_TRUE)) ch = true;
  bool th = sys && !ch;
  bool th_eq = u_streq(th, th ? mkstr(A.slab, d.thost) : Str{A.slab, 0}, lb_dns);
  if (th && !th_eq) ch = true;
  return ch;
}


GAR_HD void user_tag_effects(const DevTables &T, const Work &W, u32 i, u32 kind, Str okey, bool *keep_visible, bool *user_thost) {
  *keep_visible = true;
  *user_thost = false;
  if (!(W.derived[i] & OBJ_HAS_TAGS_ANN)) return;
  Str tags = mkstr(T.o.slab, W.ann_tags[i]);
  bool m_ok = true, o_ok = true, c_ok = true;
  u32 pos = 0;
  Str piece;
  while (next_piece(tags, &pos, &piece)) {
    TagPiece tp = tag_piece(piece);
    if (!tp.ok) continue;
    if (STREQ_LIT(tp.key, TAG_MANAGED)) m_ok = STREQ_LIT(tp.val, "true");
    else if (STREQ_LIT(tp.key, TAG_OWNER))
      o_ok = tp.val.n == 8 + okey.n && (kind == GAR_KIND_SERVICE ? lit_eq_at(tp.val, 0, "service/") : lit_eq_at(tp.val, 0, "ingress/")) &&
             streq(substr(tp.val, 8, okey.n), okey);
    else if (STREQ_LIT(tp.key, TAG_CLUSTER)) c_ok = streq(tp.val, Str{T.cluster, T.cluster_len});
    else if (STREQ_LIT(tp.key, TAG_THOST)) *user_thost = true;
  }
  *keep_visible = m_ok && o_ok && c_ok;
}
GAR_HD bool eg_contains(const DevTables &T, const AccDigest &d, Str lb_arn) {
  u32 nep = d.n_eps == 0xFFFF ? T.a.eg_ep_begin[d.eg + 1] - d.ep_begin : d.n_eps;
  for (u32 x = 0; x < nep; x++)
    if (streq(mkstr(T.a.slab, x == 0 ? d.ep0 : T.a.ep_id[d.ep_begin + x]), lb_arn)) return true;
  return false;
}
GAR_HD void ga_later_step(const DevTables &T, const Work &W, u32 i, u32 kind, Str okey, u64 okh, u32 jb, u32 j, u32 lb, u32 prev_lb, bool pending, OpSink &s, u32 *ev);

GAR_HD u32 ga_reconcile(const DevTables &T, const Work &W, u32 i, bool valid, OpSink &s) {
  const gar_objects &o = T.o;
  const gar_actual &A = T.a;
  u32 result = GAR_STATUS(GAR_ST_IGNORED, 0, 0);
  u32 dv = 0, kind = 0, jb = 0, nj = 0;
  Str okey{T.o.slab, 0};
  u64 okh = 0;
  bool ensure = false;
  if (valid) {
    dv = W.derived[i];
    if (dv & GAR_DV_GA_ELIGIBLE) {
      jb = o.obj_lbi_begin[i];
      nj = o.obj_lbi_begin[i + 1] - jb;
      kind = o.obj_kind[i];
      if (nj < 1) {
        result = GAR_STATUS(GAR_ST_SKIP_NO_LB, 0, 0);
      } else {
        okey = object_key(T, i);
        okh = W.okey_hash[i];
        if (!(dv & GAR_DV_GA_MANAGED)) {
          OwnerIter it = owner_open(W, okh, okey);
          for (u32 acc; (acc = owner_next(T, W, kind, it)) != GAR_NONE;) put_delete_chain(T, s, i, kind, acc);
          result = GAR_STATUS(GAR_ST_OK, 0, GAR_EV_DELETED);
        } else {
          ensure = true;
        }
      }
    }
  }
  u32 ev = 0;
  bool stop = false;
  u32 prev_lb = GAR_NONE;
  bool pending = false;
  for (u32 j = 0;; j++) {
    bool act = ensure && !stop && j < nj;
    if (!GAR_ANY(act)) break;
    bool probe = false;
    Str hostname{o.slab, 0}, tregion{o.slab, 0}, tname{o.slab, 0};
    if (act) {
      u32 code = W.tok_code[jb + j];
      if (code == GAR_TOK_PANIC) {
        result = GAR_STATUS(GAR_ST_PANIC, 0, ev);
        stop = true;
      } else if (code == GAR_TOK_NOT_AWS) {
      } else if (code >= GAR_TOK_ERR_NOT_ELB) {
        result = GAR_STATUS(GAR_ST_ERR_RETRY, GAR_D_NOT_ELB + (code - GAR_TOK_ERR_NOT_ELB), ev);
        stop = true;
      } else {
        probe = true;
        hostname = mkstr(o.slab, o.lbi_hostname[jb + j]);
        tregion = mkstr(o.slab, W.tok_region[jb + j]);
        tname = mkstr(o.slab, W.tok_name[jb + j]);
      }
    }
    u32 lb_state = 0;
    u32 lb = u_find_lb(T, W, probe, tregion, tname, &lb_state);
    bool have_lb = probe && lb != GAR_NONE;
    Str lb_dns = have_lb ? mkstr(A.slab, A.lb_dns[lb]) : Str{A.slab, 0};
    bool dns_eq = u_streq(have_lb, lb_dns, hostname);
    bool go = false;
    if (probe) {
      if (!have_lb) {
        result = GAR_STATUS(GAR_ST_ERR_RETRY, GAR_D_LB_NOT_FOUND, ev);
        stop = true;
      } else if (!dns_eq) {
        result = GAR_STATUS(GAR_ST_ERR_RETRY, GAR_D_LB_DNS_MISMATCH, ev);
        stop = true;
      } else if (lb_state != GAR_LB_ACTIVE) {
        result = GAR_STATUS(GAR_ST_REQUEUE_30S, 0, ev);
        stop = true;
      } else {
        go = true;
      }
    }
    const bool later = go && prev_lb != GAR_NONE;
    if (later) ga_later_step(T, W, i, kind, okey, okh, jb, j, lb, prev_lb, pending, s, &ev);
    go = go && !later;
    Cursor oc = u_open(W.ix_owner, go, okh);
    Str lb_arn = go ? mkstr(A.slab, A.lb_arn[lb]) : Str{A.slab, 0};
    u32 nacc = 0;
    for (;;) {
      u32 acc = u_owner_next(T, W, go && !stop, kind, okey, oc);
      bool a = acc != GAR_NONE;
      if (!GAR_ANY(a)) break;
      if (a) nacc++;
      AccDigest d;
      d.flags = 0;
      if (a) d = W.acc_digest[acc];
      if (u_accelerator_changed(T, W, a, i, dv, kind, acc, d, okey, lb_dns)) s.put(GAR_OP_HEAD(GAR_OP_GA_UPDATE_ACCEL, GAR_CTRL_GA, kind), i, j, acc, lb, GAR_NONE);
      u32 eg = GAR_NONE;
      if (a) {
        if (d.flags & ACCD_LIS_MANY) {
          result = GAR_STATUS(GAR_ST_ERR_RETRY, GAR_D_TOO_MANY_LISTENERS, ev);
          stop = true;
        } else if (d.flags & ACCD_LIS_NONE) {
          s.put(GAR_OP_HEAD(GAR_OP_GA_CREATE_LISTENER, GAR_CTRL_GA, kind), i, j, acc, GAR_NONE, GAR_NONE);
          s.put(GAR_OP_HEAD(GAR_OP_GA_CREATE_EG, GAR_CTRL_GA, kind), i, j, acc, GAR_NONE, lb);
        } else {
          u32 lis = d.lis;
          bool want_udp = kind == GAR_KIND_SERVICE && (dv & GAR_DV_PROTO_UDP);
          bool changed = ((d.flags & ACCD_LIS_UDP) != 0) != want_udp;
          if (!changed) {
            PortList want = desired_ports(T, W, i);
            if (d.n_ports <= 2 && want.n == d.n_ports && (d.n_ports < 1 || want.p[0] == d.port0) && (d.n_ports < 2 || (want.p[1] == d.port1 && d.port0 != d.port1))) changed = false;
            else changed = ports_changed(PortList{A.pr_from + d.pr_begin, d.n_ports == 0xFFFF ? A.lis_pr_begin[lis + 1] - d.pr_begin : d.n_ports}, want);
          }
          if (changed) s.put(GAR_OP_HEAD(GAR_OP_GA_UPDATE_LISTENER, GAR_CTRL_GA, kind), i, j, acc, lis, GAR_NONE);
          if (d.flags & ACCD_EG_MANY) {
            result = GAR_STATUS(GAR_ST_ERR_RETRY, GAR_D_TOO_MANY_EGS, ev);
            stop = true;
          } else if (d.flags & ACCD_EG_NONE) {
            s.put(GAR_OP_HEAD(GAR_OP_GA_CREATE_EG, GAR_CTRL_GA, kind), i, j, acc, lis, lb);
          } else {
            eg = d.eg;
          }
        }
      }
      bool contains = false;
      u32 nep = eg != GAR_NONE ? (d.n_eps == 0xFFFF ? A.eg_ep_begin[eg + 1] - d.ep_begin : d.n_eps) : 0;
      for (u32 x = 0;; x++) {
        bool more = !contains && x < nep;
        if (!GAR_ANY(more)) break;
        gar_str id = more ? (x == 0 ? d.ep0 : A.ep_id[d.ep_begin + x]) : 0;
        if (u_streq(more, mkstr(A.slab, id), lb_arn)) contains = true;
      }
      if (eg != GAR_NONE && !contains) s.put(GAR_OP_HEAD(GAR_OP_GA_UPDATE_EG, GAR_CTRL_GA, kind), i, j, acc, eg, lb);
    }
    if (go && !stop && nacc == 0) {
      s.put(GAR_OP_HEAD(GAR_OP_GA_CREATE_CHAIN, GAR_CTRL_GA, kind), i, j, lb, GAR_NONE, GAR_NONE);
      ev |= GAR_EV_CREATED;
      pending = true;
    }
    if ((go || later) && !stop) prev_lb = lb;
  }
  if (ensure && !stop) result = GAR_STATUS(GAR_ST_OK, 0, ev);
  return result;
}

GAR_HD void ga_later_step(const DevTables &T, const Work &W, u32 i, u32 kind, Str okey, u64 okh, u32 jb, u32 j, u32 lb, u32 prev_lb, bool pending, OpSink &s, u32 *ev) {
  const gar_actual &A = T.a;
  bool keep_visible, user_thost;
  user_tag_effects(T, W, i, kind, okey, &keep_visible, &user_thost);
  if (!keep_visible) {
    s.put(GAR_OP_HEAD(GAR_OP_GA_CREATE_CHAIN, GAR_CTRL_GA, kind), i, j, lb, GAR_NONE, GAR_NONE);
    *ev |= GAR_EV_CREATED;
    return;
  }
  Str lb_arn = mkstr(A.slab, A.lb_arn[lb]);
  const bool dns_differs = !user_thost && !streq(mkstr(A.slab, A.lb_dns[lb]), mkstr(A.slab, A.lb_dns[prev_lb]));
  const bool arn_differs = !streq(lb_arn, mkstr(A.slab, A.lb_arn[prev_lb]));
  if (pending) {
    if (dns_differs) s.put(GAR_OP_HEAD(GAR_OP_GA_UPDATE_ACCEL, GAR_CTRL_GA, kind), i, j, GAR_PENDING, lb, GAR_NONE);
    if (arn_differs) s.put(GAR_OP_HEAD(GAR_OP_GA_UPDATE_EG, GAR_CTRL_GA, kind), i, j, GAR_PENDING, GAR_PENDING, lb);
  }
  OwnerIter it = owner_open(W, okh, okey);
  for (u32 acc; (acc = owner_next(T, W, kind, it)) != GAR_NONE;) {
    if (dns_differs) s.put(GAR_OP_HEAD(GAR_OP_GA_UPDATE_ACCEL, GAR_CTRL_GA, kind), i, j, acc, lb, GAR_NONE);
    const AccDigest d = W.acc_digest[acc];
    const bool created = (d.flags & (ACCD_LIS_NONE | ACCD_EG_NONE)) != 0;
    bool replaced = created;
    for (u32 jp = 0; jp < j && !replaced; jp++) {
      if (W.tok_code[jb + jp] > GAR_TOK_NLB) continue;
      u32 st;
      u32 lbp = find_lb(T, W, mkstr(T.o.slab, W.tok_region[jb + jp]), mkstr(T.o.slab, W.tok_name[jb + jp]), &st);
      if (lbp != GAR_NONE && !eg_contains(T, d, mkstr(A.slab, A.lb_arn[lbp]))) replaced = true;
    }
    const bool contains = replaced ? !arn_differs : eg_contains(T, d, lb_arn);
    if (!contains) s.put(GAR_OP_HEAD(GAR_OP_GA_UPDATE_EG, GAR_CTRL_GA, kind), i, j, acc, created ? GAR_PENDING : d.eg, lb);
  }
}


constexpr u32 OWNED_CACHE = 8;
struct OwnedHit {
  u32 v, rec, zone;
  gar_str name;
};
struct Owned {
  OwnedHit hit[OWNED_CACHE];
  u32 n;
  u64 okh;
  u32 kind;
  Str key;
};
GAR_HD bool owned_match(const DevTables &T, const IdxEntry &e, u32 kind, Str key) {
  return (e.a1 >> 31) == kind && streq(mkstr(T.a.slab, e.s0), key);
}
GAR_HD void owned_collect(const DevTables &T, const Work &W, u64 okh, u32 kind, Str key, Owned &o) {
  o.n = 0;
  o.okh = okh;
  o.kind = kind;
  o.key = key;
  Cursor c = idx_open(W.ix_val, okh);
  IdxEntry e;
  while (idx_next(W.ix_val, c, &e)) {
    if (!owned_match(T, e, kind, key)) continue;
    if (o.n < OWNED_CACHE) o.hit[o.n] = OwnedHit{e.row, e.a0, e.a1 & 0x3FFFFFFFu, e.s1};
    o.n++;
  }
}
GAR_HD void u_owned_collect(const DevTables &T, const Work &W, bool active, u64 okh, u32 kind, Str key, Owned &o) {
  if (active) {
    o.n = 0;
    o.okh = okh;
    o.kind = kind;
    o.key = key;
  }
  Cursor c = active ? idx_open(W.ix_val, okh) : Cursor{0, 0, 0};
  for (; GAR_ANY(c.pos < c.end);) {
    IdxEntry e;
    bool hit = false;
    if (c.pos < c.end) {
      e = load_entry(W.ix_val.ent + c.pos++);
      hit = e.tag == c.tag && (e.a1 >> 31) == kind;
    }
    if (u_streq(hit, hit ? mkstr(T.a.slab, e.s0) : Str{T.a.slab, 0}, key)) {
      if (o.n < OWNED_CACHE) o.hit[o.n] = OwnedHit{e.row, e.a0, e.a1 & 0x3FFFFFFFu, e.s1};
      o.n++;
    }
  }
}
GAR_HD OwnedHit owned_get(const DevTables &T, const Work &W, const Owned &o, u32 k) {
  if (k < OWNED_CACHE) return o.hit[k];
  Cursor c = idx_open(W.ix_val, o.okh);
  IdxEntry e;
  u32 seen = 0;
  OwnedHit h{GAR_NONE, GAR_NONE, GAR_NONE, 0};
  while (idx_next(W.ix_val, c, &e)) {
    if (!owned_match(T, e, o.kind, o.key)) continue;
    if (seen++ == k) {
      h = OwnedHit{e.row, e.a0, e.a1 & 0x3FFFFFFFu, e.s1};
      break;
    }
  }
  return h;
}

GAR_HD u32 first_alias_a(const DevTables &T, const Work &W, u32 zone, Str name, u64 name_hash, gar_str *alias_dns) {
  Cursor c = idx_open(W.ix_alias, key_hash_zoned_h(zone, name_hash));
  IdxEntry e;
  while (idx_next(W.ix_alias, c, &e)) {
    if (e.a0 != zone || e.a1 != GAR_RR_A) continue;
    if (streq(mkstr(T.a.slab, e.s0), name)) {
      *alias_dns = e.s1;
      return e.row;
    }
  }
  return GAR_NONE;
}
GAR_HD u32 next_alias_any(const DevTables &T, const Work &W, u32 zone, Str name, u32 after ) {
  Cursor c = idx_open(W.ix_alias, key_hash_zoned(zone, name));
  IdxEntry e;
  while (idx_next(W.ix_alias, c, &e)) {
    if (after != GAR_NONE && e.row <= after) continue;
    if (e.a0 != zone) continue;
    if (streq(mkstr(T.a.slab, e.s0), name)) return e.row;
  }
  return GAR_NONE;
}

GAR_HD void r53_cleanup(const DevTables &T, const Work &W, u32 obj, u32 kind, const Owned &ow, OpSink &s) {
  const gar_actual &A = T.a;
  u32 head = GAR_OP_HEAD(GAR_OP_R53_DELETE_RECORD, GAR_CTRL_R53, obj == GAR_NONE ? 0 : kind);
  u32 k = 0;
  while (k < ow.n) {
    u32 zone = owned_get(T, W, ow, k).zone;
    u32 kend = k;
    while (kend < ow.n && owned_get(T, W, ow, kend).zone == zone) kend++;
    u32 last = GAR_NONE;
    for (;;) {
      u32 best = GAR_NONE, best_v = GAR_NONE;
      for (u32 x = k; x < kend; x++) {
        OwnedHit h = owned_get(T, W, ow, x);
        u32 r = next_alias_any(T, W, zone, mkstr(A.slab, h.name), last);
        if (r != GAR_NONE && (best == GAR_NONE || r < best)) {
          best = r;
          best_v = h.v;
        }
      }
      if (best == GAR_NONE) break;
      s.put(head, obj, 0, zone, best, best_v);
      last = best;
    }
    for (u32 x = k; x < kend; x++) {
      OwnedHit h = owned_get(T, W, ow, x);
      s.put(head, obj, 1, zone, h.rec, h.v);
    }
    k = kend;
  }
}

GAR_HD bool piece_seen_before(Str all, Str hn) {
  u32 pos = 0;
  Str piece;
  while (next_piece(all, &pos, &piece)) {
    if (piece.p >= hn.p) return false;
    if (streq(piece, hn)) return true;
  }
  return false;
}

GAR_HD u32 r53_reconcile(const DevTables &T, const Work &W, u32 i, bool valid, OpSink &s) {
  const gar_objects &o = T.o;
  const gar_actual &A = T.a;
  u32 result = GAR_STATUS(GAR_ST_IGNORED, 0, 0);
  u32 kind = 0, jb = 0, nj = 0;
  Str okey{T.o.slab, 0}, hostnames{T.o.slab, 0};
  u64 okh = 0;
  bool ensure = false;
  Owned ow;
  ow.n = 0;
  if (valid) {
    u32 dv = W.derived[i];
    if (dv & GAR_DV_R53_ELIGIBLE) {
      kind = o.obj_kind[i];
      okey = object_key(T, i);
      okh = W.okey_hash[i];
      if (!(dv & GAR_DV_R53_ANNOTATED)) {
        owned_collect(T, W, okh, kind, okey, ow);
        r53_cleanup(T, W, i, kind, ow, s);
        result = GAR_STATUS(GAR_ST_OK, 0, GAR_EV_DELETED);
      } else {
        ensure = true;
        hostnames = mkstr(o.slab, W.ann_r53[i]);
        jb = o.obj_lbi_begin[i];
        nj = o.obj_lbi_begin[i + 1] - jb;
      }
    }
  }
  u32 ev = 0;
  bool stop = false, collected = false;
  bool have_prev = false;
  Str prev_acc_dns{A.slab, 0};
  for (u32 j = 0;; j++) {
    bool act = ensure && !stop && j < nj;
    if (!GAR_ANY(act)) break;
    bool probe = false;
    Str lbhost{o.slab, 0};
    if (act) {
      u32 code = W.tok_code[jb + j];
      if (code == GAR_TOK_PANIC) {
        result = GAR_STATUS(GAR_ST_PANIC, 0, ev);
        stop = true;
      } else if (code == GAR_TOK_NOT_AWS) {
      } else if (code >= GAR_TOK_ERR_NOT_ELB) {
        result = GAR_STATUS(GAR_ST_ERR_RETRY, GAR_D_NOT_ELB + (code - GAR_TOK_ERR_NOT_ELB), ev);
        stop = true;
      } else {
        probe = true;
        lbhost = mkstr(o.slab, o.lbi_hostname[jb + j]);
      }
    }
    u32 acc = GAR_NONE;
    gar_str acc_dns_ref = 0;
    u32 nacc = u_find_by_hostname(T, W, probe, lbhost, &acc, &acc_dns_ref);
    bool go = false;
    if (probe) {
      if (nacc > 1) {
        result = GAR_STATUS(GAR_ST_REQUEUE_60S, GAR_D_ACCEL_MANY, ev);
        stop = true;
      } else if (nacc == 0) {
        result = GAR_STATUS(GAR_ST_REQUEUE_60S, GAR_D_ACCEL_NONE, ev);
        stop = true;
      } else {
        go = true;
      }
    }
    Str acc_dns = go ? mkstr(A.slab, acc_dns_ref) : Str{A.slab, 0};
    if (GAR_ANY(go && !collected)) {
      u_owned_collect(T, W, go && !collected, okh, kind, okey, ow);
      if (go) collected = true;
    }
    bool created = false;
    u32 pos = 0, k = 0;
    for (;;) {
      bool more = go && !stop && pos <= hostnames.n;
      if (!GAR_ANY(more)) break;
      u32 comma = u_find_byte(more, hostnames, pos, ',');
      Str hn = more ? substr(hostnames, pos, comma - pos) : Str{o.slab, 0};
      pos = comma + 1;
      u32 zone = u_find_hosted_zone(T, W, more, hn);
      if (more && zone == GAR_NONE) {
        result = GAR_STATUS(GAR_ST_ERR_RETRY, GAR_D_NO_HOSTED_ZONE, ev);
        stop = true;
        more = false;
      }
      u32 rec = GAR_NONE;
      gar_str rec_alias = 0;
      for (u32 x = 0;; x++) {
        bool has = more && x < ow.n;
        if (!GAR_ANY(has)) break;
        Str nm{A.slab, 0};
        bool inzone = false;
        if (has) {
          OwnedHit h = owned_get(T, W, ow, x);
          inzone = h.zone == zone;
          if (inzone) nm = mkstr(A.slab, h.name);
        }
        bool cand = u_record_name_matches(inzone, nm, hn);
        gar_str al = 0;
        u32 r = u_first_alias_a(T, W, cand, zone, nm, &al);
        if (cand && r != GAR_NONE && (rec == GAR_NONE || r < rec)) {
          rec = r;
          rec_alias = al;
        }
      }
      bool have = more && rec != GAR_NONE;
      Str al = have ? mkstr(A.slab, rec_alias) : Str{A.slab, 0};
      bool shape = have && al.n == acc_dns.n + 1 && al.p[al.n - 1] == '.';
      bool same = u_streq(shape, substr(al, 0, shape ? acc_dns.n : 0), acc_dns);
      if (more) {
        if (!piece_seen_before(hostnames, hn)) {
          if (!have_prev) {
            if (rec == GAR_NONE) {
              s.put(GAR_OP_HEAD(GAR_OP_R53_CREATE, GAR_CTRL_R53, kind), i, GAR_R53_SUB(j, k), zone, acc, GAR_NONE);
              created = true;
            } else if (!same) {
              s.put(GAR_OP_HEAD(GAR_OP_R53_UPSERT_A, GAR_CTRL_R53, kind), i, GAR_R53_SUB(j, k), zone, acc, rec);
            }
          } else if (!streq(acc_dns, prev_acc_dns)) {
            s.put(GAR_OP_HEAD(GAR_OP_R53_UPSERT_A, GAR_CTRL_R53, kind), i, GAR_R53_SUB(j, k), zone, acc, rec == GAR_NONE ? GAR_PENDING : rec);
          }
        }
        k++;
      }
    }
    if (go && !stop && created) ev |= GAR_EV_CREATED;
    if (go && !stop) {
      have_prev = true;
      prev_acc_dns = acc_dns;
    }
  }
  if (ensure && !stop) result = GAR_STATUS(GAR_ST_OK, 0, ev);
  return result;
}


GAR_HD void link_value_alias(const DevTables &T, const Work &W, u32 v) {
  u32 row = GAR_NONE;
  gar_str dns = 0;
  if (W.val_cls[v] != VAL_NOT_OWNER) {
    u32 rec = W.val_rec[v];
    row = first_alias_a(T, W, W.rec_zone[rec], mkstr(T.a.slab, T.a.rec_name[rec]), W.rec_name_hash[rec], &dns);
  }
  ValLink l;
  l.alias_row = row;
  l.pad = 0;
  l.alias_dns = dns;
  W.val_link[v] = l;
}

GAR_HD void r53_prepare(const DevTables &T, const Work &W, u32 i, u32 t, bool valid, u32 *status) {
  const gar_objects &o = T.o;
  u32 mode = R53_MODE_DONE, st = GAR_STATUS(GAR_ST_IGNORED, 0, 0), npairs = 0;
  bool probe = false;
  Str lbhost{o.slab, 0}, hostnames{o.slab, 0};
  if (valid) {
    u32 dv = W.derived[i];
    if (dv & GAR_DV_R53_ELIGIBLE) {
      u32 jb = o.obj_lbi_begin[i], nj = o.obj_lbi_begin[i + 1] - jb;
      if (!(dv & GAR_DV_R53_ANNOTATED) || nj > 1) {
        mode = R53_MODE_OBJECT;
      } else if (nj == 0) {
        st = GAR_STATUS(GAR_ST_OK, 0, 0);
      } else {
        u32 code = W.tok_code[jb];
        if (code == GAR_TOK_PANIC) st = GAR_STATUS(GAR_ST_PANIC, 0, 0);
        else if (code == GAR_TOK_NOT_AWS) st = GAR_STATUS(GAR_ST_OK, 0, 0);
        else if (code >= GAR_TOK_ERR_NOT_ELB) st = GAR_STATUS(GAR_ST_ERR_RETRY, GAR_D_NOT_ELB + (code - GAR_TOK_ERR_NOT_ELB), 0);
        else {
          probe = true;
          lbhost = mkstr(o.slab, o.lbi_hostname[jb]);
          hostnames = mkstr(o.slab, W.ann_r53[i]);
        }
      }
    }
  }
  u32 acc = GAR_NONE;
  gar_str acc_dns = 0;
  u32 nacc = u_find_by_hostname(T, W, probe, lbhost, &acc, &acc_dns);
  bool go = false;
  if (probe) {
    if (nacc > 1) st = GAR_STATUS(GAR_ST_REQUEUE_60S, GAR_D_ACCEL_MANY, 0);
    else if (nacc == 0) st = GAR_STATUS(GAR_ST_REQUEUE_60S, GAR_D_ACCEL_NONE, 0);
    else go = true;
  }
  u32 pos = 0;
  for (;;) {
    bool more = go && pos <= hostnames.n;
    if (!GAR_ANY(more)) break;
    u32 comma = u_find_byte(more, hostnames, pos, ',');
    if (more) {
      npairs++;
      pos = comma + 1;
    }
  }
  if (go) mode = R53_MODE_PAIRS;
  if (valid) {
    W.r53_mode[i] = (u8)mode;
    W.r53_acc[i] = acc;
    W.r53_acc_dns[i] = acc_dns;
    W.pair_begin[t] = npairs;
    if (mode == R53_MODE_DONE) status[t] = st;
  }
}

GAR_HD void r53_fill_pairs(const DevTables &T, const Work &W, u32 i, u32 t) {
  if (W.r53_mode[i] != R53_MODE_PAIRS) return;
  gar_str ref = W.ann_r53[i];
  Str hostnames = mkstr(T.o.slab, ref);
  u32 p = W.pair_begin[t], pos = 0, np = 0;
  u32 st[8], ln[8];
  Str piece;
  while (next_piece(hostnames, &pos, &piece)) {
    if (p >= W.pair_cap) break;
    W.pair_obj[p] = i;
    W.pair_hn[p] = GAR_STR(GAR_STR_OFF(ref) + (u64)(piece.p - hostnames.p), piece.n);
    bool repeat = false;
    for (u32 q = 0; q < np && q < 8 && !repeat; q++) repeat = ln[q] == piece.n && streq(substr(hostnames, st[q], ln[q]), piece);
    if (!repeat && np > 8) repeat = piece_seen_before(hostnames, piece);
    W.pair_code[p] = repeat ? (u8)PAIR_REPEAT : (u8)PAIR_IN_SYNC;
    if (np < 8) {
      st[np] = (u32)(piece.p - hostnames.p);
      ln[np] = piece.n;
    }
    np++;
    p++;
  }
}

GAR_HD void r53_pair(const DevTables &T, const Work &W, u32 p, bool valid) {
  const gar_actual &A = T.a;
  u32 i = 0, kind = 0;
  Str hn{T.o.slab, 0}, okey{T.o.slab, 0};
  u64 okh = 0;
  valid = valid && W.pair_code[p] != PAIR_REPEAT;
  if (valid) {
    i = W.pair_obj[p];
    hn = mkstr(T.o.slab, W.pair_hn[p]);
    kind = T.o.obj_kind[i];
    okey = object_key(T, i);
    okh = W.okey_hash[i];
  }
  u32 zone = u_find_hosted_zone(T, W, valid, hn);
  bool live = valid && zone != GAR_NONE;
  u32 rec = GAR_NONE;
  gar_str rec_alias = 0;
  Cursor c = u_open(W.ix_val, live, okh);
  for (; GAR_ANY(c.pos < c.end);) {
    IdxEntry e;
    bool hit = false;
    if (c.pos < c.end) {
      e = load_entry(W.ix_val.ent + c.pos++);
      hit = e.tag == c.tag && (e.a1 >> 31) == kind && (e.a1 & 0x3FFFFFFFu) == zone;
    }
    bool mine = u_streq(hit, hit ? mkstr(A.slab, e.s0) : Str{A.slab, 0}, okey);
    Str nm = mine ? mkstr(A.slab, e.s1) : Str{A.slab, 0};
    bool plain = mine && !(e.a1 & VALNAME_HAS_BACKSLASH);
    bool shape = plain && nm.n == hn.n + 1 && nm.p[nm.n - 1] == '.';
    bool match = u_streq(shape, substr(nm, 0, shape ? hn.n : 0), hn);
    if (mine && !plain) match = record_name_matches(nm, hn);
    if (match) {
      ValLink l = W.val_link[e.row];
      if (l.alias_row != GAR_NONE && (rec == GAR_NONE || l.alias_row < rec)) {
        rec = l.alias_row;
        rec_alias = l.alias_dns;
      }
    }
  }
  bool have = live && rec != GAR_NONE;
  Str acc_dns = have ? mkstr(A.slab, W.r53_acc_dns[i]) : Str{A.slab, 0};
  Str al = have ? mkstr(A.slab, rec_alias) : Str{A.slab, 0};
  bool shape = have && al.n == acc_dns.n + 1 && al.p[al.n - 1] == '.';
  bool same = u_streq(shape, substr(al, 0, shape ? acc_dns.n : 0), acc_dns);
  if (valid) {
    u32 code = !live ? PAIR_NO_ZONE : rec == GAR_NONE ? PAIR_CREATE : same ? PAIR_IN_SYNC : PAIR_UPSERT;
    W.pair_code[p] = (u8)code;
    W.pair_zone[p] = zone;
    W.pair_rec[p] = rec;
  }
}

GAR_HD u32 r53_combine(const DevTables &T, const Work &W, u32 i, u32 t, bool valid, u32 prev_status, OpSink &s) {
  u32 mode = valid ? W.r53_mode[i] : R53_MODE_DONE;
  u32 st = prev_status;
  bool slow = mode == R53_MODE_OBJECT;
  if (GAR_ANY(slow)) {
    u32 r = r53_reconcile(T, W, i, slow, s);
    if (slow) st = r;
  }
  if (mode == R53_MODE_PAIRS) {
    u32 kind = T.o.obj_kind[i], acc = W.r53_acc[i];
    bool created = false, stop = false;
    u32 k = 0;
    for (u32 p = W.pair_begin[t]; p < W.pair_begin[t + 1] && p < W.pair_cap && !stop; p++, k++) {
      u32 code = W.pair_code[p];
      if (code == PAIR_NO_ZONE) {
        st = GAR_STATUS(GAR_ST_ERR_RETRY, GAR_D_NO_HOSTED_ZONE, 0);
        stop = true;
      } else if (code == PAIR_CREATE) {
        s.put(GAR_OP_HEAD(GAR_OP_R53_CREATE, GAR_CTRL_R53, kind), i, GAR_R53_SUB(0, k), W.pair_zone[p], acc, GAR_NONE);
        created = true;
      } else if (code == PAIR_UPSERT) {
        s.put(GAR_OP_HEAD(GAR_OP_R53_UPSERT_A, GAR_CTRL_R53, kind), i, GAR_R53_SUB(0, k), W.pair_zone[p], acc, W.pair_rec[p]);
      }
    }
    if (!stop) st = GAR_STATUS(GAR_ST_OK, 0, created ? GAR_EV_CREATED : 0);
  }
  return st;
}


GAR_HD bool object_in_cache(const DevTables &T, const Work &W, u32 kind, Str key, u64 key_hash) {
  Cursor c = idx_open(W.ix_obj, key_hash);
  IdxEntry e;
  while (idx_next(W.ix_obj, c, &e))
    if (e.a0 == kind && streq(mkstr(T.o.slab, e.s0), key)) return true;
  return false;
}

GAR_HD u32 ga_orphan(const DevTables &T, const Work &W, u32 acc, OpSink &s) {
  if (acc >= W.acc_guest_from) return 0;
  if (W.acc_claimed && W.acc_claimed[acc]) return 0;
  u32 fl = W.acc_flags[acc];
  if (!(fl & ACC_MINE) || !(fl & ACC_OWNER_3PART)) return 0;
  u32 kind = (fl & ACC_OWNER_INGRESS) ? 1u : 0u;
  if (object_in_cache(T, W, kind, mkstr(T.a.slab, W.acc_owner_key[acc]), W.acc_owner_hash[acc])) return 0;
  put_delete_chain(T, s, GAR_NONE, 0, acc);
  return 1;
}

GAR_HD void mark_orphan_value(const DevTables &T, const Work &W, u32 v) {
  u32 cls = W.val_cls[v];
  u8 orphan = 0;
  if (cls & VAL_OWNER_3PART) {
    u32 kind = (cls & VAL_OWNER_INGRESS) ? 1u : 0u;
    orphan = object_in_cache(T, W, kind, mkstr(T.a.slab, W.val_key[v]), W.val_key_hash[v]) ? 0 : 1;
  }
  if (orphan) {
    u32 rec = W.val_rec[v];
    ix_count(W.hist[IX_OVN], key_hash_zoned_h(W.rec_zone[rec], W.rec_name_hash[rec]));
  }
  W.val_orphan[v] = orphan;
}

GAR_HD void r53_orphan_alias(const DevTables &T, const Work &W, u32 r, OpSink &s) {
  const gar_actual &A = T.a;
  if (!A.rec_has_alias[r]) return;
  u32 zone = W.rec_zone[r];
  Str name = mkstr(A.slab, A.rec_name[r]);
  u64 h = key_hash_zoned_h(zone, W.rec_name_hash[r]);
  Cursor c = idx_open(W.ix_ovn, h);
  IdxEntry e;
  while (idx_next(W.ix_ovn, c, &e)) {
    if (e.a1 != zone || !streq(mkstr(A.slab, e.s0), name)) continue;
    Str val = mkstr(A.slab, e.s1);
    bool dup = false;
    Cursor c2 = idx_open(W.ix_ovn, h);
    IdxEntry e2;
    while (idx_next(W.ix_ovn, c2, &e2) && e2.row < e.row) {
      if (e2.a1 == zone && streq(mkstr(A.slab, e2.s0), name) && streq(mkstr(A.slab, e2.s1), val)) {
        dup = true;
        break;
      }
    }
    if (dup) continue;
    s.put(GAR_OP_HEAD(GAR_OP_R53_DELETE_RECORD, GAR_CTRL_R53, 0), GAR_NONE, 0, zone, r, e.row);
  }
}


struct DevBindings {
  gar_bindings b;
  HashIdx ix_eg;
};

GAR_HD bool egb_eg_exists(const DevBindings &B, Str arn) {
  Cursor c = idx_open(B.ix_eg, gar_hash(arn));
  IdxEntry e;
  while (idx_next(B.ix_eg, c, &e))
    if (streq(mkstr(B.b.slab, e.s0), arn)) return true;
  return false;
}

GAR_HD u32 egb_lb_of(const DevTables &T, const Work &W, u32 lbi_row, u32 *detail) {
  u32 code = W.tok_code[lbi_row];
  *detail = 0;
  if (code == GAR_TOK_NOT_AWS || code == GAR_TOK_PANIC) {
    *detail = GAR_D_NOT_ELB;
    return GAR_NONE;
  }
  if (code >= GAR_TOK_ERR_NOT_ELB) {
    *detail = GAR_D_NOT_ELB + (code - GAR_TOK_ERR_NOT_ELB);
    return GAR_NONE;
  }
  u32 st;
  u32 lb = find_lb(T, W, mkstr(T.o.slab, W.tok_region[lbi_row]), mkstr(T.o.slab, W.tok_name[lbi_row]), &st);
  if (lb == GAR_NONE) *detail = GAR_D_LB_NOT_FOUND;
  return lb;
}

GAR_HD u32 egb_reconcile(const DevTables &T, const Work &W, const DevBindings &B, u32 k, OpSink &s) {
  const gar_bindings &b = B.b;
  const gar_actual &A = T.a;
  u32 flags = b.egb_flags[k];
  u32 eb = b.egb_ep_begin[k], n = b.egb_ep_begin[k + 1] - eb;
  Str eg_arn = mkstr(b.slab, b.egb_eg_arn[k]);
  auto H = [](u32 op) { return GAR_OP_HEAD(op, GAR_CTRL_EGB, 0); };
  if (flags & GAR_EGB_DELETING) {
    if (n == 0 || !egb_eg_exists(B, eg_arn)) {
      s.put(H(GAR_OP_EGB_REMOVE_FINALIZER), k, 0, GAR_NONE, GAR_NONE, GAR_NONE);
      return GAR_STATUS(GAR_ST_OK, 0, 0);
    }
    u32 len = n;
    for (u32 i = 0; i < n; i++) {
      u32 src = 2 * i < n - 1 ? 2 * i : n - 1;
      s.put(H(GAR_OP_EGB_REMOVE_ENDPOINT), k, 0, eb + src, GAR_NONE, GAR_NONE);
      if (i + 1 > len) return GAR_STATUS(GAR_ST_PANIC, 0, 0);
      len--;
    }
    s.put(H(GAR_OP_EGB_UPDATE_STATUS), k, 0, GAR_NONE, GAR_NONE, GAR_NONE);
    return GAR_STATUS(GAR_ST_REQUEUE_1S, 0, 0);
  }
  if (!(flags & GAR_EGB_HAS_FINALIZERS)) {
    s.put(H(GAR_OP_EGB_ADD_FINALIZER), k, 0, GAR_NONE, GAR_NONE, GAR_NONE);
    return GAR_STATUS(GAR_ST_OK, 0, 0);
  }
  u32 jb = 0, nj = 0;
  u32 refkind = b.egb_ref_kind[k];
  if (refkind != GAR_EGB_REF_NONE) {
    u32 kind = refkind == GAR_EGB_REF_SERVICE ? GAR_KIND_SERVICE : GAR_KIND_INGRESS;
    Str key = mkstr(b.slab, b.egb_ref_key[k]);
    Cursor c = idx_open(W.ix_obj, key_hash_kinded(kind, key));
    IdxEntry e;
    u32 obj = GAR_NONE;
    while (idx_next(W.ix_obj, c, &e))
      if (e.a0 == kind && streq(mkstr(T.o.slab, e.s0), key)) {
        obj = e.row;
        break;
      }
    if (obj == GAR_NONE) return GAR_STATUS(GAR_ST_ERR_RETRY, GAR_D_REF_NOT_FOUND, 0);
    jb = T.o.obj_lbi_begin[obj];
    nj = T.o.obj_lbi_begin[obj + 1] - jb;
  }
  for (u32 j = 0; j < nj; j++) {
    u32 detail;
    if (egb_lb_of(T, W, jb + j, &detail) == GAR_NONE) return GAR_STATUS(GAR_ST_ERR_RETRY, detail, 0);
  }
  auto arn_of = [&](u32 j) {
    u32 d;
    return mkstr(A.slab, A.lb_arn[egb_lb_of(T, W, jb + j, &d)]);
  };
  auto is_first = [&](u32 j) {
    Str a = arn_of(j);
    for (u32 i = 0; i < j; i++)
      if (streq(arn_of(i), a)) return false;
    return true;
  };
  auto in_status = [&](Str a) {
    for (u32 x = 0; x < n; x++)
      if (streq(mkstr(b.slab, b.ep_id[eb + x]), a)) return true;
    return false;
  };
  auto in_arns = [&](Str id) {
    for (u32 j = 0; j < nj; j++)
      if (streq(arn_of(j), id)) return true;
    return false;
  };
  u32 nnew = 0, nrem = 0;
  for (u32 j = 0; j < nj; j++)
    if (is_first(j) && !in_status(arn_of(j))) nnew++;
  for (u32 x = 0; x < n; x++)
    if (!in_arns(mkstr(b.slab, b.ep_id[eb + x]))) nrem++;
  if (nnew == 0 && nrem == 0 && (flags & GAR_EGB_OBSERVED)) return GAR_STATUS(GAR_ST_OK, 0, 0);
  if (!egb_eg_exists(B, eg_arn)) return GAR_STATUS(GAR_ST_ERR_RETRY, GAR_D_EG_NOT_FOUND, 0);
  if (nrem > 0 && nj == 0) return GAR_STATUS(GAR_ST_PANIC, 0, 0);
  for (u32 x = 0; x < n; x++)
    if (!in_arns(mkstr(b.slab, b.ep_id[eb + x]))) s.put(H(GAR_OP_EGB_REMOVE_ENDPOINT), k, 0, eb + x, GAR_NONE, GAR_NONE);
  Str last_region = nj ? mkstr(T.o.slab, W.tok_region[jb + nj - 1]) : Str{T.o.slab, 0};
  for (u32 j = 0; j < nj; j++) {
    if (!is_first(j) || in_status(arn_of(j))) continue;
    u32 jl = j;
    for (u32 i = j + 1; i < nj; i++)
      if (streq(arn_of(i), arn_of(j))) jl = i;
    u32 st;
    u32 lb2 = find_lb(T, W, last_region, mkstr(T.o.slab, W.tok_name[jb + jl]), &st);
    if (lb2 == GAR_NONE) return GAR_STATUS(GAR_ST_ERR_RETRY, GAR_D_LB_NOT_FOUND, 0);
    if (st != GAR_LB_ACTIVE) return GAR_STATUS(GAR_ST_REQUEUE_30S, 0, 0);
    s.put(H(GAR_OP_EGB_ADD_ENDPOINT), k, 0, lb2, GAR_NONE, GAR_NONE);
  }
  for (u32 j = 0; j < nj; j++)
    if (is_first(j)) {
      u32 d;
      s.put(H(GAR_OP_EGB_UPDATE_WEIGHT), k, 0, egb_lb_of(T, W, jb + j, &d), GAR_NONE, GAR_NONE);
    }
  s.put(H(GAR_OP_EGB_UPDATE_STATUS), k, 0, GAR_NONE, GAR_NONE, GAR_NONE);
  return GAR_STATUS(GAR_ST_OK, 0, 0);
}
```

Before: 165.4 million.

## Resolve accelerator and value owners to objects once via per-object segments

Each value and accelerator is resolved to its owning object through the object index once. The results are bucketed into per-object segments (accelerators, then values), so the GA and Route53 passes walk a contiguous owned list instead of probing the owner and value hash indexes with repeated string compares. Duplicate object keys are canonicalised during bucket ordering, and the owner and value indexes are built lazily only when something still needs them. This adds extra placement, scan and sort kernels plus new buffers, and makes the change-set depend on the canonicalisation being correct.

```diff
diff --git a/aws-global-accelerator-controller_b200/csrc/gar_pipeline.h b/aws-global-accelerator-controller_b200/csrc/gar_pipeline.h
--- a/aws-global-accelerator-controller_b200/csrc/gar_pipeline.h
+++ b/aws-global-accelerator-controller_b200/csrc/gar_pipeline.h
@@ -23,7 +23,8 @@
   S_IX_LB, S_IX_OWNER = S_IX_LB + 3, S_IX_THOST = S_IX_OWNER + 3, S_IX_ZONE = S_IX_THOST + 3, S_IX_VAL = S_IX_ZONE + 3,
   S_IX_ALIAS = S_IX_VAL + 3, S_IX_OBJ = S_IX_ALIAS + 3, S_IX_OVN = S_IX_OBJ + 3,
   S_SORT_KEYS = S_IX_OVN + 3, S_SORT_VALS, S_SORT_KEYS_ALT, S_SORT_VALS_ALT, S_SORT_TAGS,
-  S_COUNTS, S_STATUS_GA, S_STATUS_R53, S_OPS, S_ERRFLAG, S_IX_EG, S_IX_EG_ENT, S_IX_EG_PAD, S_ACC_CLAIMED,
+  S_COUNTS, S_STATUS_GA, S_STATUS_R53, S_OPS, S_ERRFLAG, S_IX_EG, S_IX_EG_ENT, S_IX_EG_PAD,
+  S_VAL_OBJ, S_ACC_OBJ, S_OBJ_CANON, S_OWN_BEGIN, S_OWN_FILL, S_OWN_ENT, S_OWN_MULTI,
   S_IXA_BEGIN, S_IXA_FILL, S_IXA_ENT, S_IXA_MULTI, S_OVN_FILL, S_OVN_MULTI, S_LB_HASH, S_REC_FLAGS,
   S_NSLOTS
 };
@@ -37,6 +38,7 @@
   u32 *errflag;
   GAR_HD void operator()(u32 i) const {
     classify_object(T, W, i);
+    W.obj_canon[i] = i;
     u32 dv = W.derived[i];
     if (dv & OBJ_KEY_BAD) GAR_ATOMIC_ADD(errflag, 1u);
     derived_public[i] = dv & 0xFFu;
@@ -314,6 +316,14 @@
 };
 
 constexpr u32 IDX_SMALL_BUCKET = 48;
+struct CanonHook {
+  u32 *canon;
+  const u8 *slab;
+  u32 b0, b1;
+  GAR_HD void operator()(u32 b, const IdxEntry *ent, u32 lo, u32 m) const {
+    if (canon && b >= b0 && b < b1) canon_bucket(ent, lo, m, slab, canon);
+  }
+};
 template <class RowF>
 struct FIdxRows {
   RowF rowf;
@@ -357,6 +367,7 @@
   const u32 *begin;
   IdxEntry *ent;
   u32 *overflow;
+  CanonHook canon;
   GAR_HD void operator()(u32 b) const {
     u32 lo = begin[b], m = begin[b + 1] - lo;
     if (m < 2) return;
@@ -373,6 +384,7 @@
       }
       if (j != k) ent[lo + j] = x;
     }
+    canon(b, ent, lo, m);
   }
 };
 struct FIdxGather {
@@ -382,6 +394,15 @@
   IdxEntry *ent;
   GAR_HD void operator()(u32 p) const {
     if (p < *nvalid) ent[p] = tmp[vals[p]];
+  }
+};
+struct FIdxCanon {
+  const u32 *begin;
+  const IdxEntry *ent;
+  CanonHook canon;
+  GAR_HD void operator()(u32 b) const {
+    const u32 lo = begin[b], m = begin[b + 1] - lo;
+    if (m >= 2) canon(b, ent, lo, m);
   }
 };
 template <class RowF>
@@ -430,6 +451,7 @@
   IdxEntry *ent;
   const u32 *multi;
   u32 *overflow;
+  CanonHook canon;
   GAR_HD void operator()(u32 t) const {
     const u32 b = multi[1 + t];
     const u32 lo = begin[b], m = begin[b + 1] - lo;
@@ -446,6 +468,7 @@
       }
       if (j != k) ent[lo + j] = x;
     }
+    canon(b, ent, lo, m);
   }
 };
 enum FlagWord { FW_BAD_KEYS = 0, FW_IDX_OVERFLOW = 1, FW_NDPORTS = 2, FW_NPAIRS = 3, FW_SEC0 = 4 , FW_WORDS = 16 };
@@ -478,13 +501,77 @@
   Work W;
   GAR_HD void operator()(u32 v) const {
     link_value_alias(T, W, v);
-    mark_orphan_value(T, W, v);
-  }
-};
-struct FMarkOrphanValue {
-  DevTables T;
-  Work W;
-  GAR_HD void operator()(u32 v) const { mark_orphan_value(T, W, v); }
+    resolve_value(T, W, v);
+  }
+};
+struct FResolveValue {
+  DevTables T;
+  Work W;
+  GAR_HD void operator()(u32 v) const { resolve_value(T, W, v); }
+};
+struct FResolveAccel {
+  DevTables T;
+  Work W;
+  GAR_HD void operator()(u32 a) const { resolve_accel(T, W, a); }
+};
+GAR_HD IdxEntry own_entry(const DevTables &T, const Work &W, u32 x) {
+  IdxEntry e;
+  e.tag = e.a0 = e.a1 = 0;
+  e.s0 = e.s1 = 0;
+  if (x < T.a.n_accels) {
+    e.row = x;
+    return e;
+  }
+  const u32 v = x - T.a.n_accels, rec = W.val_rec[v];
+  const ValLink l = W.val_link[v];
+  e.tag = l.alias_row;
+  e.row = v;
+  e.a0 = rec;
+  e.a1 = W.rec_zone[rec] | ((W.rec_flags[rec] & 1) ? VALNAME_HAS_BACKSLASH : 0u);
+  e.s0 = l.alias_dns;
+  e.s1 = T.a.rec_name[rec];
+  return e;
+}
+GAR_HD u32 own_segment(const DevTables &T, const Work &W, u32 x) {
+  const u32 nacc = T.a.n_accels;
+  const u32 o = x < nacc ? W.acc_obj[x] : W.val_obj[x - nacc];
+  return o == GAR_NONE ? 2 * T.o.n_objects : 2 * o + (x < nacc ? 0u : 1u);
+}
+struct FOwnPlace {
+  DevTables T;
+  Work W;
+  u32 *cursor;
+  IdxEntry *ent;
+  u32 x0;
+  GAR_HD void operator()(u32 i) const {
+    const u32 x = x0 + i, k = own_segment(T, W, x);
+    if (k == 2 * T.o.n_objects) return;
+#if defined(__CUDA_ARCH__)
+    const u32 pos = atomicAdd(&cursor[k], 1u);
+#else
+    const u32 pos = cursor[k]++;
+#endif
+    ent[pos] = own_entry(T, W, x);
+  }
+};
+struct FOwnKeys {
+  DevTables T;
+  Work W;
+  u32 *keys, *vals;
+  GAR_HD void operator()(u32 x) const {
+    keys[x] = own_segment(T, W, x);
+    vals[x] = x;
+  }
+};
+struct FOwnGather {
+  DevTables T;
+  Work W;
+  const u32 *vals;
+  const u32 *total;
+  IdxEntry *ent;
+  GAR_HD void operator()(u32 p) const {
+    if (p < *total) ent[p] = own_entry(T, W, vals[p]);
+  }
 };
 
 struct CountLayout {
@@ -742,7 +829,7 @@
   explicit Pipeline(B &b, const DevTables &t) : be(b), T(t) {}
 
   template <class RowF>
-  HashIdx build_index(int slot, u32 nrows, u32 load, RowF rowf, u32 *overflow, bool force_radix) {
+  HashIdx build_index(int slot, u32 nrows, u32 load, RowF rowf, u32 *overflow, bool force_radix, CanonHook canon = {}) {
     u32 nb = next_pow2(nrows / load < 16 ? 16 : nrows / load);
     u32 *keys = (u32 *)be.ensure(S_SORT_KEYS, sizeof(u32) * (size_t)(nrows + 1));
     u32 *vals = (u32 *)be.ensure(S_SORT_VALS, sizeof(u32) * (size_t)(nrows + 1));
@@ -756,12 +843,13 @@
       u32 *cursor = (u32 *)be.ensure(S_SORT_KEYS_ALT, sizeof(u32) * (size_t)(nb + 1));
       be.copy32(cursor, begin, nb);
       be.for_each("idx_place", nrows, FIdxPlace{keys, cursor, tmp, ent, nb});
-      be.for_each("idx_order", nb, FIdxOrder{begin, ent, overflow});
+      be.for_each("idx_order", nb, FIdxOrder{begin, ent, overflow, canon});
     } else if (nrows) {
       u32 *keys2 = (u32 *)be.ensure(S_SORT_KEYS_ALT, sizeof(u32) * (size_t)(nrows + 1));
       u32 *vals2 = (u32 *)be.ensure(S_SORT_VALS_ALT, sizeof(u32) * (size_t)(nrows + 1));
       be.sort_pairs(keys, vals, keys2, vals2, nrows, ilog2(nb) + 1);
       be.for_each("idx_gather", nrows, FIdxGather{vals, begin + nb, tmp, ent});
+      if (canon.canon) be.for_each("idx_order", nb, FIdxCanon{begin, ent, canon});
     }
     return HashIdx{begin, ent, nb - 1};
   }
@@ -790,7 +878,9 @@
     W.r53_mode = (u8 *)be.ensure(S_R53_MODE, (size_t)n + 1);
     W.r53_acc = (u32 *)be.ensure(S_R53_ACC, 4 * (size_t)(n + 1));
     W.r53_acc_dns = (gar_str *)be.ensure(S_R53_ACC_DNS, 8 * (size_t)(n + 1));
-  }
+    W.obj_canon = (u32 *)be.ensure(S_OBJ_CANON, 4 * (size_t)(n + 1));
+  }
+  CanonHook canon_hook(u32 b0, u32 b1) const { return CanonHook{W.obj_canon, T.o.slab, b0, b1}; }
   void alloc_work() {
     const u32 nacc = T.a.n_accels, nrec = T.a.n_records, nval = T.a.n_values;
     alloc_obj_work();
@@ -808,6 +898,8 @@
     W.val_cls = (u8 *)be.ensure(S_VAL_CLS, nval + 1);
     W.val_key = (gar_str *)be.ensure(S_VAL_KEY, 8 * (size_t)(nval + 1));
     W.val_orphan = (u8 *)be.ensure(S_VAL_ORPHAN, nval + 1);
+    W.val_obj = (u32 *)be.ensure(S_VAL_OBJ, 4 * (size_t)(nval + 1));
+    W.acc_obj = (u32 *)be.ensure(S_ACC_OBJ, 4 * (size_t)(nacc + 1));
     W.val_link = (ValLink *)be.ensure(S_VAL_LINK, sizeof(ValLink) * (size_t)(nval + 1));
     W.acc_digest = (AccDigest *)be.ensure(S_ACC_DIGEST, sizeof(AccDigest) * (size_t)(nacc + 1));
     W.lb_hash = (u64 *)be.ensure(S_LB_HASH, 8 * (size_t)(T.a.n_lbs + 1));
@@ -819,7 +911,6 @@
     be.fill32(errflag, 0, FW_WORDS);
     W.acc_guest_from = acc_guest_from;
     W.sharded = sharded;
-    W.acc_claimed = nullptr;
   }
   void stage1() {
     const u32 n = T.o.n_objects, nlbi = T.o.n_lbi, nacc = T.a.n_accels, nrec = T.a.n_records, nval = T.a.n_values;
@@ -887,36 +978,76 @@
     be.fill32(ixa_multi, 0, 1);
     const IxPlan &P = planA;
     auto n = [&](int k) { return P.want[k] ? P.rows[k] : 0u; };
-    be.for_each_multi("idx_place", {n(IX_LB), n(IX_OWNER), n(IX_THOST), n(IX_ZONE), n(IX_VAL), n(IX_ALIAS), n(IX_OBJ), P.total_nb},
-                      placer(IX_LB, FRowLb{T, W}), placer(IX_OWNER, FRowOwner{T, W}), placer(IX_THOST, FRowThost{T, W}), placer(IX_ZONE, FRowZone{T}),
-                      placer(IX_VAL, FRowVal{T, W}), placer(IX_ALIAS, FRowAlias{T, W}), placer(IX_OBJ, FRowObj{T, W}), FIdxMultiList{ixa_begin, ixa_multi});
-    be.for_each_dyn("idx_order", ixa_multi, multi_cap, FIdxOrderMulti{ixa_begin, ixa_ent, ixa_multi, overflow});
+    be.for_each_multi("idx_place", {n(IX_LB), n(IX_THOST), n(IX_ZONE), n(IX_ALIAS), n(IX_OBJ), P.total_nb},
+                      placer(IX_LB, FRowLb{T, W}), placer(IX_THOST, FRowThost{T, W}), placer(IX_ZONE, FRowZone{T}),
+                      placer(IX_ALIAS, FRowAlias{T, W}), placer(IX_OBJ, FRowObj{T, W}), FIdxMultiList{ixa_begin, ixa_multi});
+    const CanonHook canon = P.want[IX_OBJ] ? canon_hook(P.off[IX_OBJ], P.off[IX_OBJ] + P.nb[IX_OBJ]) : CanonHook{};
+    be.for_each_dyn("idx_order", ixa_multi, multi_cap, FIdxOrderMulti{ixa_begin, ixa_ent, ixa_multi, overflow, canon});
     if (P.want[IX_LB]) W.ix_lb = group_a_index(IX_LB);
-    if (P.want[IX_OWNER]) W.ix_owner = group_a_index(IX_OWNER);
     if (P.want[IX_THOST]) W.ix_thost = group_a_index(IX_THOST);
     if (P.want[IX_ZONE]) W.ix_zone = group_a_index(IX_ZONE);
-    if (P.want[IX_VAL]) W.ix_val = group_a_index(IX_VAL);
     if (P.want[IX_ALIAS]) W.ix_alias = group_a_index(IX_ALIAS);
     if (P.want[IX_OBJ]) W.ix_obj = group_a_index(IX_OBJ);
   }
-  void arm_ovn() {
-    ovn_nb = next_pow2(T.a.n_values / 8 < 16 ? 16 : T.a.n_values / 8);
-    u32 *cnt = (u32 *)be.ensure(S_IX_OVN + 0, 4 * (size_t)(ovn_nb + 2));
-    be.fill32(cnt, 0, (size_t)ovn_nb + 2);
-    W.hist[IX_OVN] = IxHist{cnt, ovn_nb - 1};
-  }
-  void finish_ovn() {
-    const u32 nval = T.a.n_values;
-    u32 *begin = W.hist[IX_OVN].cnt;
-    be.exclusive_scan(begin, ovn_nb + 1);
-    u32 *cursor = (u32 *)be.ensure(S_OVN_FILL, 4 * (size_t)(ovn_nb + 1));
-    IdxEntry *ent = (IdxEntry *)be.ensure(S_IX_OVN + 1, sizeof(IdxEntry) * (size_t)(nval + 1));
-    u32 *multi = (u32 *)be.ensure(S_OVN_MULTI, 4 * (size_t)(nval / 2 + 3));
-    be.copy32(cursor, begin, (size_t)ovn_nb + 1);
-    be.fill32(multi, 0, 1);
-    be.for_each_multi("idx_place", {nval, ovn_nb}, FIdxPlaceDirect<FRowOvn>{FRowOvn{T, W}, cursor, ent, ovn_nb - 1}, FIdxMultiList{begin, multi});
-    be.for_each_dyn("idx_order", multi, nval / 2 + 1, FIdxOrderMulti{begin, ent, multi, errflag + FW_IDX_OVERFLOW});
-    W.ix_ovn = HashIdx{begin, ent, ovn_nb - 1};
+  void resolve_owners(bool link_aliases) {
+    const u32 n = T.o.n_objects, nacc = T.a.n_accels, nval = T.a.n_values, nseg = 2 * n;
+    u32 *overflow = errflag + FW_IDX_OVERFLOW;
+    W.own_begin = (u32 *)be.ensure(S_OWN_BEGIN, 4 * (size_t)(nseg + 2));
+    be.fill32(W.own_begin, 0, (size_t)nseg + 1);
+    u32 *ovn = nullptr;
+    if (!force_radix) {
+      ovn_nb = next_pow2(nval / 8 < 16 ? 16 : nval / 8);
+      ovn = (u32 *)be.ensure(S_IX_OVN + 0, 4 * (size_t)(ovn_nb + 2));
+      be.fill32(ovn, 0, (size_t)ovn_nb + 2);
+      W.hist[IX_OVN] = IxHist{ovn, ovn_nb - 1};
+    } else {
+      W.hist[IX_OVN] = IxHist{nullptr, 0};
+    }
+    if (link_aliases) be.for_each_multi("value_joins", {nval, nacc}, FValueJoins{T, W}, FResolveAccel{T, W});
+    else be.for_each_multi("resolve_owners", {nval, nacc}, FResolveValue{T, W}, FResolveAccel{T, W});
+    be.exclusive_scan(W.own_begin, nseg + 1);
+    IdxEntry *own = (IdxEntry *)be.ensure(S_OWN_ENT, sizeof(IdxEntry) * ((size_t)nacc + nval + 1));
+    if (!force_radix) {
+      be.exclusive_scan(ovn, ovn_nb + 1);
+      u32 *ovn_cursor = (u32 *)be.ensure(S_OVN_FILL, 4 * (size_t)(ovn_nb + 1));
+      IdxEntry *ovn_ent = (IdxEntry *)be.ensure(S_IX_OVN + 1, sizeof(IdxEntry) * (size_t)(nval + 1));
+      u32 *ovn_multi = (u32 *)be.ensure(S_OVN_MULTI, 4 * (size_t)(nval / 2 + 3));
+      u32 *own_cursor = (u32 *)be.ensure(S_OWN_FILL, 4 * (size_t)(nseg + 1));
+      const u32 own_multi_cap = (u32)(((u64)nacc + nval) / 2 + 1);
+      u32 *own_multi = (u32 *)be.ensure(S_OWN_MULTI, 4 * (size_t)(own_multi_cap + 2));
+      be.copy32(ovn_cursor, ovn, (size_t)ovn_nb + 1);
+      be.copy32(own_cursor, W.own_begin, (size_t)nseg + 1);
+      be.fill32(ovn_multi, 0, 1);
+      be.fill32(own_multi, 0, 1);
+      be.for_each_multi("idx_place", {nval, ovn_nb, nacc, nval, nseg}, FIdxPlaceDirect<FRowOvn>{FRowOvn{T, W}, ovn_cursor, ovn_ent, ovn_nb - 1},
+                        FIdxMultiList{ovn, ovn_multi}, FOwnPlace{T, W, own_cursor, own, 0}, FOwnPlace{T, W, own_cursor, own, nacc},
+                        FIdxMultiList{W.own_begin, own_multi});
+      be.for_each_dyn("idx_order", ovn_multi, nval / 2 + 1, FIdxOrderMulti{ovn, ovn_ent, ovn_multi, overflow});
+      be.for_each_dyn("idx_order", own_multi, own_multi_cap, FIdxOrderMulti{W.own_begin, own, own_multi, overflow});
+      W.ix_ovn = HashIdx{ovn, ovn_ent, ovn_nb - 1};
+    } else {
+      const u32 nx = nacc + nval;
+      u32 *keys = (u32 *)be.ensure(S_SORT_KEYS, 4 * (size_t)(nx + 1));
+      u32 *vals = (u32 *)be.ensure(S_SORT_VALS, 4 * (size_t)(nx + 1));
+      u32 *keys2 = (u32 *)be.ensure(S_SORT_KEYS_ALT, 4 * (size_t)(nx + 1));
+      u32 *vals2 = (u32 *)be.ensure(S_SORT_VALS_ALT, 4 * (size_t)(nx + 1));
+      if (nx) {
+        be.for_each("own_keys", nx, FOwnKeys{T, W, keys, vals});
+        be.sort_pairs(keys, vals, keys2, vals2, nx, ilog2(nseg + 1) + 1);
+        be.for_each("own_gather", nx, FOwnGather{T, W, vals, W.own_begin + nseg, own});
+      }
+      W.ix_ovn = build_index(S_IX_OVN, nval, 8, FRowOvn{T, W}, overflow, true);
+    }
+    W.own = own;
+    owners_stale = false;
+  }
+  bool owner_indexes = false;
+  void build_owner_indexes() {
+    if (owner_indexes) return;
+    u32 *overflow = errflag + FW_IDX_OVERFLOW;
+    W.ix_owner = build_index(S_IX_OWNER, T.a.n_accels, 1, FRowOwner{T, W}, overflow, force_radix);
+    W.ix_val = build_index(S_IX_VAL, T.a.n_values, 1, FRowVal{T, W}, overflow, force_radix);
+    owner_indexes = true;
   }
 
   void prepare_route() {
@@ -938,32 +1069,25 @@
   u64 ops_cap = 0;
   bool tiny_caps = false;
   int prepare() {
-    const u32 n = T.o.n_objects, nacc = T.a.n_accels, nzone = T.a.n_zones, nrec = T.a.n_records, nval = T.a.n_values;
+    const u32 n = T.o.n_objects, nacc = T.a.n_accels, nzone = T.a.n_zones, nrec = T.a.n_records;
     alloc_work();
-    if (!force_radix) {
-      arm_group_a((1u << IX_OVN) - 1);
-      arm_ovn();
-    }
+    if (!force_radix) arm_group_a((1u << IX_LB) | (1u << IX_THOST) | (1u << IX_ZONE) | (1u << IX_ALIAS) | (1u << IX_OBJ));
     stage1();
     listen_ports();
 
     u32 *overflow = errflag + FW_IDX_OVERFLOW;
     if (!force_radix) {
       finish_group_a();
-      if (nval) be.for_each("value_joins", nval, FValueJoins{T, W});
-      finish_ovn();
     } else {
       W.ix_lb = build_index(S_IX_LB, T.a.n_lbs, 1, FRowLb{T, W}, overflow, true);
-      W.ix_owner = build_index(S_IX_OWNER, nacc, 1, FRowOwner{T, W}, overflow, true);
       W.ix_thost = build_index(S_IX_THOST, nacc, 1, FRowThost{T, W}, overflow, true);
       W.ix_zone = build_index(S_IX_ZONE, nzone, 1, FRowZone{T}, overflow, true);
-      W.ix_val = build_index(S_IX_VAL, nval, 1, FRowVal{T, W}, overflow, true);
       W.ix_alias = build_index(S_IX_ALIAS, nrec, 2, FRowAlias{T, W}, overflow, true);
-      W.ix_obj = build_index(S_IX_OBJ, n, 1, FRowObj{T, W}, overflow, true);
-      if (nval) be.for_each("value_joins", nval, FValueJoins{T, W});
-      W.ix_ovn = build_index(S_IX_OVN, nval, 8, FRowOvn{T, W}, overflow, true);
-    }
-    obj_stale = ovn_stale = false;
+      W.ix_obj = build_index(S_IX_OBJ, n, 1, FRowObj{T, W}, overflow, true, canon_hook(0, 0xFFFFFFFFu));
+    }
+    resolve_owners(true);
+    obj_stale = false;
+    owner_indexes = false;
     return GAR_OK;
   }
   void listen_ports() {
@@ -978,7 +1102,7 @@
     if (n) be.for_each("listen_ports_write", n, FJsonWrite{T, W});
   }
 
-  bool obj_stale = false, ovn_stale = false;
+  bool obj_stale = false, owners_stale = false;
   void prepare_objects() {
     const u32 n = T.o.n_objects, nlbi = T.o.n_lbi;
     alloc_obj_work();
@@ -988,22 +1112,9 @@
     if (n) be.for_each("classify_objects", n, FClassify{T, W, derived_public, nullptr, errflag});
     if (nlbi) be.for_each_staged("tokenise_hostnames", nlbi, FTokenise{T, W});
     listen_ports();
-    W.ix_obj = build_index(S_IX_OBJ, n, 1, FRowObj{T, W}, errflag + FW_IDX_OVERFLOW, force_radix);
+    W.ix_obj = build_index(S_IX_OBJ, n, 1, FRowObj{T, W}, errflag + FW_IDX_OVERFLOW, force_radix, canon_hook(0, 0xFFFFFFFFu));
     obj_stale = false;
-    ovn_stale = true;
-  }
-  void prepare_orphan_values() {
-    const u32 nval = T.a.n_values;
-    if (!force_radix) {
-      arm_ovn();
-      if (nval) be.for_each("orphan_values", nval, FMarkOrphanValue{T, W});
-      finish_ovn();
-    } else {
-      W.hist[IX_OVN] = IxHist{nullptr, 0};
-      if (nval) be.for_each("orphan_values", nval, FMarkOrphanValue{T, W});
-      W.ix_ovn = build_index(S_IX_OVN, nval, 8, FRowOvn{T, W}, errflag + FW_IDX_OVERFLOW, true);
-    }
-    ovn_stale = false;
+    owners_stale = true;
   }
   int index_objects() {
     for (int attempt = 0; attempt < 2; attempt++) {
@@ -1052,8 +1163,6 @@
     gar_op *stage_r53 = (gar_op *)be.ensure(S_STAGE_R53, sizeof(gar_op) * ((size_t)n * OPS_STAGE_CAP + 1));
     u32 *st_ga = (u32 *)be.out_status_ga(n);
     u32 *st_r53 = (u32 *)be.out_status_r53(n);
-    W.acc_claimed = (u8 *)be.ensure(S_ACC_CLAIMED, (size_t)nacc + 4);
-    be.fill32((u32 *)W.acc_claimed, 0, ((size_t)nacc + 3) / 4);
     if (n) be.for_each_warp("ga_objects", n, FGaObj{T, W, counts + L.ga_obj(0), stage_ga, st_ga, nullptr});
     r53_relational(n, nullptr, st_r53);
     if (n) be.for_each_warp("r53_objects", n, FR53Obj{T, W, counts + L.r53_obj(0), stage_r53, st_r53, nullptr});
@@ -1072,7 +1181,6 @@
     if (orphan_sweep)
       be.for_each_multi("orphans_emit", {nacc, nrec, nval}, FGaOrphan{T, W, L, counts, ops, cap}, FR53OrphanAlias{T, W, L, counts, ops, cap},
                         FR53OrphanValue{T, W, L, counts, ops, cap});
-    W.acc_claimed = nullptr;
     return GAR_OK;
   }
 
@@ -1087,6 +1195,7 @@
     u32 *st_ga = (u32 *)be.out_status_ga(m);
     u32 *st_r53 = (u32 *)be.out_status_r53(m);
     u32 *derived_out = (u32 *)be.out_derived_keys(m);
+    if (nd) build_owner_indexes();
     if (m) {
       be.for_each("gather_derived", m, FGatherDerived{W.derived, rows, derived_out});
       be.for_each_warp("ga_objects", m, FGaObj{T, W, c_ga, stage_ga, st_ga, rows});
@@ -1132,7 +1241,7 @@
     for (int attempt = 0; attempt < 8; attempt++) {
       u64 sig = 0;
       if (full) {
-        sig = hmix(hmix(prepared ? (obj_stale || ovn_stale ? 9 : 1) : 2, force_radix ? 3 : 4), hmix(hmix(dport_cap, pair_cap), ops_cap));
+        sig = hmix(hmix(prepared ? (obj_stale || owners_stale ? 9 : 1) : 2, force_radix ? 3 : 4), hmix(hmix(dport_cap, pair_cap), ops_cap));
         sig = hmix(sig, hmix(orphan_sweep ? 5 : 6, tiny_caps ? 7 : 8)) | 1;
       }
       const int g = full ? be.graph_begin(sig) : 0;
@@ -1140,7 +1249,7 @@
       if (g != 2) {
         if (!prepared) rc = prepare();
         else if (obj_stale) prepare_objects();
-        if (rc == GAR_OK && full && ovn_stale) prepare_orphan_values();
+        if (rc == GAR_OK && owners_stale) resolve_owners(false);
         if (rc == GAR_OK) rc = decide();
       }
       prepared = true;
diff --git a/aws-global-accelerator-controller_b200/csrc/gar_rows.h b/aws-global-accelerator-controller_b200/csrc/gar_rows.h
--- a/aws-global-accelerator-controller_b200/csrc/gar_rows.h
+++ b/aws-global-accelerator-controller_b200/csrc/gar_rows.h
@@ -109,7 +109,11 @@
   ValLink *val_link;
   u32 acc_guest_from;
   u32 sharded;
-  u8 *acc_claimed;
+  u32 *val_obj;
+  u32 *acc_obj;
+  u32 *obj_canon;
+  u32 *own_begin;
+  const IdxEntry *own;
   u8 *r53_mode;
   u32 *r53_acc;
   gar_str *r53_acc_dns;
@@ -434,6 +438,18 @@
   return GAR_NONE;
 }
 
+struct OwnRange {
+  u32 pos, end;
+};
+GAR_HD OwnRange own_accs(const Work &W, u32 i) {
+  const u32 s = 2 * W.obj_canon[i];
+  return OwnRange{W.own_begin[s], W.own_begin[s + 1]};
+}
+GAR_HD OwnRange own_vals(const Work &W, u32 i) {
+  const u32 s = 2 * W.obj_canon[i] + 1;
+  return OwnRange{W.own_begin[s], W.own_begin[s + 1]};
+}
+
 struct OwnerIter {
   Cursor c;
   Str key;
@@ -530,18 +546,6 @@
       *state = e.a0;
     }
   }
-  return found;
-}
-
-GAR_HD u32 u_owner_next(const DevTables &T, const Work &W, bool active, u32 kind, Str key, Cursor &c) {
-  u32 found = GAR_NONE;
-  U_BUCKET_LOOP(active && found == GAR_NONE, c) {
-    IdxEntry e;
-    bool hit = u_bucket_step(W.ix_owner, active && found == GAR_NONE, c, &e);
-    hit = hit && (((e.a0 & ACC_OWNER_INGRESS) != 0) ? 1u : 0u) == kind;
-    if (u_streq(hit, mkstr(T.a.slab, e.s0), key)) found = e.row;
-  }
-  if (found != GAR_NONE && W.acc_claimed) W.acc_claimed[found] = 1;
   return found;
 }
 
@@ -814,7 +818,7 @@
     if (streq(mkstr(T.a.slab, x == 0 ? d.ep0 : T.a.ep_id[d.ep_begin + x]), lb_arn)) return true;
   return false;
 }
-GAR_HD void ga_later_step(const DevTables &T, const Work &W, u32 i, u32 kind, Str okey, u64 okh, u32 jb, u32 j, u32 lb, u32 prev_lb, bool pending, OpSink &s, u32 *ev);
+GAR_HD void ga_later_step(const DevTables &T, const Work &W, u32 i, u32 kind, Str okey, u32 jb, u32 j, u32 lb, u32 prev_lb, bool pending, OpSink &s, u32 *ev);
 
 GAR_HD u32 ga_reconcile(const DevTables &T, const Work &W, u32 i, bool valid, OpSink &s) {
   const gar_objects &o = T.o;
@@ -822,7 +826,6 @@
   u32 result = GAR_STATUS(GAR_ST_IGNORED, 0, 0);
   u32 dv = 0, kind = 0, jb = 0, nj = 0;
   Str okey{T.o.slab, 0};
-  u64 okh = 0;
   bool ensure = false;
   if (valid) {
     dv = W.derived[i];
@@ -834,10 +837,9 @@
         result = GAR_STATUS(GAR_ST_SKIP_NO_LB, 0, 0);
       } else {
         okey = object_key(T, i);
-        okh = W.okey_hash[i];
         if (!(dv & GAR_DV_GA_MANAGED)) {
-          OwnerIter it = owner_open(W, okh, okey);
-          for (u32 acc; (acc = owner_next(T, W, kind, it)) != GAR_NONE;) put_delete_chain(T, s, i, kind, acc);
+          const OwnRange ar = own_accs(W, i);
+          for (u32 p = ar.pos; p < ar.end; p++) put_delete_chain(T, s, i, kind, W.own[p].row);
           result = GAR_STATUS(GAR_ST_OK, 0, GAR_EV_DELETED);
         } else {
           ensure = true;
@@ -891,15 +893,15 @@
       }
     }
     const bool later = go && prev_lb != GAR_NONE;
-    if (later) ga_later_step(T, W, i, kind, okey, okh, jb, j, lb, prev_lb, pending, s, &ev);
+    if (later) ga_later_step(T, W, i, kind, okey, jb, j, lb, prev_lb, pending, s, &ev);
     go = go && !later;
-    Cursor oc = u_open(W.ix_owner, go, okh);
+    OwnRange oc = go ? own_accs(W, i) : OwnRange{0, 0};
     Str lb_arn = go ? mkstr(A.slab, A.lb_arn[lb]) : Str{A.slab, 0};
     u32 nacc = 0;
     for (;;) {
-      u32 acc = u_owner_next(T, W, go && !stop, kind, okey, oc);
-      bool a = acc != GAR_NONE;
+      bool a = go && !stop && oc.pos < oc.end;
       if (!GAR_ANY(a)) break;
+      u32 acc = a ? W.own[oc.pos++].row : GAR_NONE;
       if (a) nacc++;
       AccDigest d;
       d.flags = 0;
@@ -954,7 +956,7 @@
   return result;
 }
 
-GAR_HD void ga_later_step(const DevTables &T, const Work &W, u32 i, u32 kind, Str okey, u64 okh, u32 jb, u32 j, u32 lb, u32 prev_lb, bool pending, OpSink &s, u32 *ev) {
+GAR_HD void ga_later_step(const DevTables &T, const Work &W, u32 i, u32 kind, Str okey, u32 jb, u32 j, u32 lb, u32 prev_lb, bool pending, OpSink &s, u32 *ev) {
   const gar_actual &A = T.a;
   bool keep_visible, user_thost;
   user_tag_effects(T, W, i, kind, okey, &keep_visible, &user_thost);
@@ -970,8 +972,9 @@
     if (dns_differs) s.put(GAR_OP_HEAD(GAR_OP_GA_UPDATE_ACCEL, GAR_CTRL_GA, kind), i, j, GAR_PENDING, lb, GAR_NONE);
     if (arn_differs) s.put(GAR_OP_HEAD(GAR_OP_GA_UPDATE_EG, GAR_CTRL_GA, kind), i, j, GAR_PENDING, GAR_PENDING, lb);
   }
-  OwnerIter it = owner_open(W, okh, okey);
-  for (u32 acc; (acc = owner_next(T, W, kind, it)) != GAR_NONE;) {
+  const OwnRange ar = own_accs(W, i);
+  for (u32 p = ar.pos; p < ar.end; p++) {
+    const u32 acc = W.own[p].row;
     if (dns_differs) s.put(GAR_OP_HEAD(GAR_OP_GA_UPDATE_ACCEL, GAR_CTRL_GA, kind), i, j, acc, lb, GAR_NONE);
     const AccDigest d = W.acc_digest[acc];
     const bool created = (d.flags & (ACCD_LIS_NONE | ACCD_EG_NONE)) != 0;
@@ -988,11 +991,21 @@
 }
 
 
-constexpr u32 OWNED_CACHE = 8;
 struct OwnedHit {
   u32 v, rec, zone;
   gar_str name;
 };
+GAR_HD OwnedHit owned_hit(const IdxEntry &e) { return OwnedHit{e.row, e.a0, e.a1 & 0x3FFFFFFFu, e.s1}; }
+struct OwnedList {
+  const IdxEntry *e;
+  u32 n;
+};
+GAR_HD OwnedList owned_list(const Work &W, u32 i) {
+  const OwnRange r = own_vals(W, i);
+  return OwnedList{W.own + r.pos, r.end - r.pos};
+}
+GAR_HD OwnedHit owned_get(const DevTables &, const Work &, const OwnedList &o, u32 k) { return owned_hit(load_entry(o.e + k)); }
+constexpr u32 OWNED_CACHE = 8;
 struct Owned {
   OwnedHit hit[OWNED_CACHE];
   u32 n;
@@ -1012,29 +1025,8 @@
   IdxEntry e;
   while (idx_next(W.ix_val, c, &e)) {
     if (!owned_match(T, e, kind, key)) continue;
-    if (o.n < OWNED_CACHE) o.hit[o.n] = OwnedHit{e.row, e.a0, e.a1 & 0x3FFFFFFFu, e.s1};
+    if (o.n < OWNED_CACHE) o.hit[o.n] = owned_hit(e);
     o.n++;
-  }
-}
-GAR_HD void u_owned_collect(const DevTables &T, const Work &W, bool active, u64 okh, u32 kind, Str key, Owned &o) {
-  if (active) {
-    o.n = 0;
-    o.okh = okh;
-    o.kind = kind;
-    o.key = key;
-  }
-  Cursor c = active ? idx_open(W.ix_val, okh) : Cursor{0, 0, 0};
-  for (; GAR_ANY(c.pos < c.end);) {
-    IdxEntry e;
-    bool hit = false;
-    if (c.pos < c.end) {
-      e = load_entry(W.ix_val.ent + c.pos++);
-      hit = e.tag == c.tag && (e.a1 >> 31) == kind;
-    }
-    if (u_streq(hit, hit ? mkstr(T.a.slab, e.s0) : Str{T.a.slab, 0}, key)) {
-      if (o.n < OWNED_CACHE) o.hit[o.n] = OwnedHit{e.row, e.a0, e.a1 & 0x3FFFFFFFu, e.s1};
-      o.n++;
-    }
   }
 }
 GAR_HD OwnedHit owned_get(const DevTables &T, const Work &W, const Owned &o, u32 k) {
@@ -1046,7 +1038,7 @@
   while (idx_next(W.ix_val, c, &e)) {
     if (!owned_match(T, e, o.kind, o.key)) continue;
     if (seen++ == k) {
-      h = OwnedHit{e.row, e.a0, e.a1 & 0x3FFFFFFFu, e.s1};
+      h = owned_hit(e);
       break;
     }
   }
@@ -1076,7 +1068,8 @@
   return GAR_NONE;
 }
 
-GAR_HD void r53_cleanup(const DevTables &T, const Work &W, u32 obj, u32 kind, const Owned &ow, OpSink &s) {
+template <class OwnedT>
+GAR_HD void r53_cleanup(const DevTables &T, const Work &W, u32 obj, u32 kind, const OwnedT &ow, OpSink &s) {
   const gar_actual &A = T.a;
   u32 head = GAR_OP_HEAD(GAR_OP_R53_DELETE_RECORD, GAR_CTRL_R53, obj == GAR_NONE ? 0 : kind);
   u32 k = 0;
@@ -1122,20 +1115,15 @@
   const gar_actual &A = T.a;
   u32 result = GAR_STATUS(GAR_ST_IGNORED, 0, 0);
   u32 kind = 0, jb = 0, nj = 0;
-  Str okey{T.o.slab, 0}, hostnames{T.o.slab, 0};
-  u64 okh = 0;
+  Str hostnames{T.o.slab, 0};
   bool ensure = false;
-  Owned ow;
-  ow.n = 0;
+  OwnedList ow{W.own, 0};
   if (valid) {
     u32 dv = W.derived[i];
     if (dv & GAR_DV_R53_ELIGIBLE) {
       kind = o.obj_kind[i];
-      okey = object_key(T, i);
-      okh = W.okey_hash[i];
       if (!(dv & GAR_DV_R53_ANNOTATED)) {
-        owned_collect(T, W, okh, kind, okey, ow);
-        r53_cleanup(T, W, i, kind, ow, s);
+        r53_cleanup(T, W, i, kind, owned_list(W, i), s);
         result = GAR_STATUS(GAR_ST_OK, 0, GAR_EV_DELETED);
       } else {
         ensure = true;
@@ -1146,7 +1134,7 @@
     }
   }
   u32 ev = 0;
-  bool stop = false, collected = false;
+  bool stop = false;
   bool have_prev = false;
   Str prev_acc_dns{A.slab, 0};
   for (u32 j = 0;; j++) {
@@ -1184,10 +1172,7 @@
       }
     }
     Str acc_dns = go ? mkstr(A.slab, acc_dns_ref) : Str{A.slab, 0};
-    if (GAR_ANY(go && !collected)) {
-      u_owned_collect(T, W, go && !collected, okh, kind, okey, ow);
-      if (go) collected = true;
-    }
+    if (go) ow = owned_list(W, i);
     bool created = false;
     u32 pos = 0, k = 0;
     for (;;) {
@@ -1348,41 +1333,33 @@
 
 GAR_HD void r53_pair(const DevTables &T, const Work &W, u32 p, bool valid) {
   const gar_actual &A = T.a;
-  u32 i = 0, kind = 0;
-  Str hn{T.o.slab, 0}, okey{T.o.slab, 0};
-  u64 okh = 0;
+  u32 i = 0;
+  Str hn{T.o.slab, 0};
   valid = valid && W.pair_code[p] != PAIR_REPEAT;
   if (valid) {
     i = W.pair_obj[p];
     hn = mkstr(T.o.slab, W.pair_hn[p]);
-    kind = T.o.obj_kind[i];
-    okey = object_key(T, i);
-    okh = W.okey_hash[i];
   }
   u32 zone = u_find_hosted_zone(T, W, valid, hn);
   bool live = valid && zone != GAR_NONE;
   u32 rec = GAR_NONE;
   gar_str rec_alias = 0;
-  Cursor c = u_open(W.ix_val, live, okh);
+  OwnRange c = live ? own_vals(W, i) : OwnRange{0, 0};
   for (; GAR_ANY(c.pos < c.end);) {
     IdxEntry e;
-    bool hit = false;
+    bool mine = false;
     if (c.pos < c.end) {
-      e = load_entry(W.ix_val.ent + c.pos++);
-      hit = e.tag == c.tag && (e.a1 >> 31) == kind && (e.a1 & 0x3FFFFFFFu) == zone;
-    }
-    bool mine = u_streq(hit, hit ? mkstr(A.slab, e.s0) : Str{A.slab, 0}, okey);
+      e = load_entry(W.own + c.pos++);
+      mine = (e.a1 & 0x3FFFFFFFu) == zone;
+    }
     Str nm = mine ? mkstr(A.slab, e.s1) : Str{A.slab, 0};
     bool plain = mine && !(e.a1 & VALNAME_HAS_BACKSLASH);
     bool shape = plain && nm.n == hn.n + 1 && nm.p[nm.n - 1] == '.';
     bool match = u_streq(shape, substr(nm, 0, shape ? hn.n : 0), hn);
     if (mine && !plain) match = record_name_matches(nm, hn);
-    if (match) {
-      ValLink l = W.val_link[e.row];
-      if (l.alias_row != GAR_NONE && (rec == GAR_NONE || l.alias_row < rec)) {
-        rec = l.alias_row;
-        rec_alias = l.alias_dns;
-      }
+    if (match && e.tag != GAR_NONE && (rec == GAR_NONE || e.tag < rec)) {
+      rec = e.tag;
+      rec_alias = e.s0;
     }
   }
   bool have = live && rec != GAR_NONE;
@@ -1428,32 +1405,53 @@
 }
 
 
-GAR_HD bool object_in_cache(const DevTables &T, const Work &W, u32 kind, Str key, u64 key_hash) {
+GAR_HD u32 find_object(const DevTables &T, const Work &W, u32 kind, Str key, u64 key_hash) {
   Cursor c = idx_open(W.ix_obj, key_hash);
   IdxEntry e;
   while (idx_next(W.ix_obj, c, &e))
-    if (e.a0 == kind && streq(mkstr(T.o.slab, e.s0), key)) return true;
-  return false;
+    if (e.a0 == kind && streq(mkstr(T.o.slab, e.s0), key)) return e.row;
+  return GAR_NONE;
+}
+GAR_HD void canon_bucket(const IdxEntry *ent, u32 lo, u32 m, const u8 *oslab, u32 *canon) {
+  for (u32 k = 1; k < m; k++) {
+    const IdxEntry x = ent[lo + k];
+    for (u32 j = 0; j < k; j++) {
+      const IdxEntry y = ent[lo + j];
+      if (y.tag == x.tag && y.a0 == x.a0 && streq(mkstr(oslab, y.s0), mkstr(oslab, x.s0))) {
+        canon[x.row] = y.row;
+        break;
+      }
+    }
+  }
 }
 
 GAR_HD u32 ga_orphan(const DevTables &T, const Work &W, u32 acc, OpSink &s) {
   if (acc >= W.acc_guest_from) return 0;
-  if (W.acc_claimed && W.acc_claimed[acc]) return 0;
   u32 fl = W.acc_flags[acc];
   if (!(fl & ACC_MINE) || !(fl & ACC_OWNER_3PART)) return 0;
-  u32 kind = (fl & ACC_OWNER_INGRESS) ? 1u : 0u;
-  if (object_in_cache(T, W, kind, mkstr(T.a.slab, W.acc_owner_key[acc]), W.acc_owner_hash[acc])) return 0;
+  if (W.acc_obj[acc] != GAR_NONE) return 0;
   put_delete_chain(T, s, GAR_NONE, 0, acc);
   return 1;
 }
 
-GAR_HD void mark_orphan_value(const DevTables &T, const Work &W, u32 v) {
+GAR_HD void resolve_accel(const DevTables &T, const Work &W, u32 a) {
+  const u32 fl = W.acc_flags[a];
+  u32 o = GAR_NONE;
+  if (acc_in_owner_index(W, a, fl)) {
+    o = find_object(T, W, (fl & ACC_OWNER_INGRESS) ? 1u : 0u, mkstr(T.a.slab, W.acc_owner_key[a]), W.acc_owner_hash[a]);
+    if (o != GAR_NONE) GAR_HIST_ADD(&W.own_begin[2 * o]);
+  }
+  W.acc_obj[a] = o;
+}
+GAR_HD void resolve_value(const DevTables &T, const Work &W, u32 v) {
   u32 cls = W.val_cls[v];
-  u8 orphan = 0;
-  if (cls & VAL_OWNER_3PART) {
-    u32 kind = (cls & VAL_OWNER_INGRESS) ? 1u : 0u;
-    orphan = object_in_cache(T, W, kind, mkstr(T.a.slab, W.val_key[v]), W.val_key_hash[v]) ? 0 : 1;
-  }
+  u32 o = GAR_NONE;
+  if (cls != VAL_NOT_OWNER) {
+    o = find_object(T, W, (cls & VAL_OWNER_INGRESS) ? 1u : 0u, mkstr(T.a.slab, W.val_key[v]), W.val_key_hash[v]);
+    if (o != GAR_NONE) GAR_HIST_ADD(&W.own_begin[2 * o + 1]);
+  }
+  W.val_obj[v] = o;
+  const u8 orphan = (cls & VAL_OWNER_3PART) && o == GAR_NONE ? 1 : 0;
   if (orphan) {
     u32 rec = W.val_rec[v];
     ix_count(W.hist[IX_OVN], key_hash_zoned_h(W.rec_zone[rec], W.rec_name_hash[rec]));
```

Result: faster. 177.8 million (median of 6 runs) (+7.5%).
